# Coloquinte/sleekit

Measured on AMD Instinct MI355X. Metric: Mweights/sec quantized (GPTQ 3-bit, 4096x4096 layer), higher is better.
Workload: dtype f64; 1 GPU; 8 layers 4096x4096, 8-level uniform codebook (GPTQ 3-bit), act_order=diag, damp=0.01, local-search moves=0, layer error included; distinct_inputs=8, allocator_settle_steps=15, gpu_max_hw_queues=4

## Files before the change

include/sleekit_amd.h:

```cpp
#ifndef SLEEKIT_AMD_H
#define SLEEKIT_AMD_H

#include <stddef.h>
#include <stdint.h>

#ifdef __cplusplus
extern "C" {
#endif

#define SLK_OK 0
#define SLK_E_ARG (-1)
#define SLK_E_NOT_PD (-2)
#define SLK_E_HIP (-3)
#define SLK_E_WS (-4)
#define SLK_INFO_HANDOFF_TIMEOUT 0x7fffffff

#define SLK_CB_VALUE 0
#define SLK_CB_INDEX 1
#define SLK_CB_UP 2
#define SLK_CB_DOWN 3
#define SLK_CB_INDEX16 4
#define SLK_CB_INDEX32 5

#define SLK_ORDER_NONE 0
#define SLK_ORDER_DIAG 1
#define SLK_ORDER_ERR 2
#define SLK_ORDER_SQERR 3
#define SLK_ORDER_KEYS 4

typedef void *slk_stream_t;

int slk_abi_version(void);
const char *slk_last_error(void);
int slk_set_option(const char *name, int value);
int slk_get_option(const char *name);
size_t slk_workspace_bytes(int R, int n);

int slk_codebook_apply(const float *x, size_t count, int levels, double lo, double hi, const float *table,
                       int what, void *out, slk_stream_t stream);

size_t slk_codebook_stats_workspace_bytes(void);
int slk_codebook_stats(const float *x, size_t count, int levels, double lo, double hi, const float *table, int by_position,
                       long long *counts, double *sums, double *sqerr, void *workspace, size_t ws_bytes, slk_stream_t stream);
size_t slk_sort_workspace_bytes(size_t count);
int slk_sort_f32(const float *x, size_t count, float *out, void *workspace, size_t ws_bytes, slk_stream_t stream);
int slk_unique_f32(const float *sorted, size_t count, float *out, int *n_out, void *workspace, size_t ws_bytes,
                   slk_stream_t stream);

int slk_rows_divide(const float *x, const float *scale, int R, int n, int invert, float *out,
                    slk_stream_t stream);

int slk_stack_rows(const float *const *src, int batch, int rows, int rows_padded, int cols, float fill, float *dst,
                   slk_stream_t stream);

int slk_hessian_strip_mean(const float *H, const float *mean, int n, float *out,
                           slk_stream_t stream);

int slk_hessian_patch_dead(float *H, float *W, int R, int n, void *workspace, size_t ws_bytes,
                           slk_stream_t stream);

int slk_hessian_accumulate(float *H, float *mean, const float *X, int n, int T,
                           long long count_before, void *workspace, size_t ws_bytes, slk_stream_t stream);

int slk_column_miss(const float *W, int R, int n, int levels, double lo, double hi, const float *table,
                    int squared, float *miss, slk_stream_t stream);

int slk_hessian_prepare(const float *H, int n, float damp, int order_mode, const float *miss,
                        long long *order_out, double *A, void *workspace, size_t ws_bytes,
                        slk_stream_t stream);
int slk_inverse_diag_keys(const double *U, const float *H, int n, float damp, int combined, double *keys,
                          void *workspace, size_t ws_bytes, slk_stream_t stream);
int slk_pivot_keys(const float *H, int n, float damp, double *keys, void *workspace, size_t ws_bytes,
                   slk_stream_t stream);
int slk_factor_ld(int n);
int slk_factor_load(const double *M, int n, double *A, slk_stream_t stream);

int slk_chol_inverse_upper(double *A, int n, double *U, int *info, void *workspace,
                           size_t ws_bytes, slk_stream_t stream);
int slk_chol_inverse_upper_lookahead(double *A, int n, double *U, int *info, void *workspace,
                                     size_t ws_bytes, slk_stream_t stream);
int slk_release_helpers(void);

int slk_hessian_prepare_batch(const float *const *H, int batch, int n, float damp, int order_mode,
                              long long *order_out, double *A, void *workspace, size_t ws_bytes, slk_stream_t stream);
int slk_chol_inverse_upper_batch(double *A, int batch, int n, double *U, int *info, void *workspace,
                                 size_t ws_bytes, slk_stream_t stream);
size_t slk_factor_workspace_bytes_batch(int batch, int n);

size_t slk_factor_payload_words(int n);
int slk_factor_pack(const double *U, const long long *order, const int *info, int n, void *payload,
                    slk_stream_t stream);
int slk_factor_unpack(const void *payload, int n, double *U, long long *order, int *info,
                      slk_stream_t stream);
int slk_factor_unpack_upper(const void *payload, int n, double *U, long long *order, int *info,
                            slk_stream_t stream);
int slk_factor_unpack_upper_batch(const void *const *payloads, int batch, int n, double *U, long long *order, int *info,
                                  int *verdict, slk_stream_t stream);

#define SLK_LOOP_UNSCALE 1
#define SLK_LOOP_LATENCY 2
int slk_gptq_quantize(const float *W, const float *scale, const long long *order, const double *U,
                      int R, int n, int levels, double lo, double hi, const float *table, int min_block,
                      int num_blocks, int flags, float *Q, uint8_t *idx, float *E_out, void *workspace,
                      size_t ws_bytes, slk_stream_t stream);

int slk_gptq_quantize_batch(const float *W, const float *scale, const long long *order, const double *U,
                            int batch, int rows_per_layer, int n, int levels, double lo, double hi,
                            const float *table, int min_block, int num_blocks, int flags, float *Q,
                            uint8_t *idx, float *E_out, void *workspace, size_t ws_bytes, slk_stream_t stream);
size_t slk_workspace_bytes_batch(int batch, int rows_per_layer, int n);

int slk_gptq_quantize_batch_error(const float *W, const float *scale, const long long *order, const double *U,
                                  const float *const *H, float damp, int batch, int rows_per_layer, int n, int levels,
                                  double lo, double hi, const float *table, int min_block, int num_blocks, int flags,
                                  float *Q, uint8_t *idx, float *E_out, float *row_err, void *workspace, size_t ws_bytes,
                                  slk_stream_t stream);

int slk_gptq_quantize_grouped(const float *W, const float *gscale, int group_size, const long long *order, const double *U,
                              int R, int n, int levels, double lo, double hi, const float *table, int min_block,
                              int num_blocks, int flags, float *Q, uint8_t *idx, float *E_out, void *workspace,
                              size_t ws_bytes, slk_stream_t stream);
int slk_gptq_quantize_grouped_batch(const float *W, const float *gscale, int group_size, const long long *order, const double *U,
                                    int batch, int rows_per_layer, int n, int levels, double lo, double hi, const float *table,
                                    int min_block, int num_blocks, int flags, float *Q, uint8_t *idx, float *E_out,
                                    void *workspace, size_t ws_bytes, slk_stream_t stream);
int slk_column_miss_grouped(const float *W, const float *gscale, int group_size, int R, int n, int levels, double lo,
                            double hi, const float *table, int squared, float *miss, slk_stream_t stream);
int slk_scale_search_grouped(const float *W, const float *base, const float *factors, int n_factors, const float *hdiag,
                             int group_size, int R, int n, int levels, double lo, double hi, const float *table, float *out,
                             slk_stream_t stream);
int slk_dequantize_grouped(const uint8_t *idx, const float *gscale, int group_size, int R, int n, int levels, double lo,
                           double hi, const float *table, float *Q, slk_stream_t stream);

int slk_gptq_quantize_grouped_asym(const float *W, const float *gscale, const float *goffset, int group_size, const long long *order,
                                   const double *U, int R, int n, int levels, double lo, double hi, const float *table,
                                   int min_block, int num_blocks, int flags, float *Q, uint8_t *idx, float *E_out,
                                   void *workspace, size_t ws_bytes, slk_stream_t stream);
int slk_gptq_quantize_grouped_asym_batch(const float *W, const float *gscale, const float *goffset, int group_size,
                                         const long long *order, const double *U, int batch, int rows_per_layer, int n,
                                         int levels, double lo, double hi, const float *table, int min_block, int num_blocks,
                                         int flags, float *Q, uint8_t *idx, float *E_out, void *workspace, size_t ws_bytes,
                                         slk_stream_t stream);
int slk_column_miss_grouped_asym(const float *W, const float *gscale, const float *goffset, int group_size, int R, int n,
                                 int levels, double lo, double hi, const float *table, int squared, float *miss,
                                 slk_stream_t stream);
int slk_dequantize_grouped_asym(const uint8_t *idx, const float *gscale, const float *goffset, int group_size, int R, int n,
                                int levels, double lo, double hi, const float *table, float *Q, slk_stream_t stream);
int slk_group_midpoints(const float *W, int group_size, int R, int n, float *goffset, float *Wc, slk_stream_t stream);
int slk_group_center(const float *W, const float *goffset, int group_size, int R, int n, float *Wc, slk_stream_t stream);

#define SLK_DTYPE_F32 0
#define SLK_DTYPE_BF16 1
#define SLK_DTYPE_F16 2
int slk_pack_indices(const uint8_t *idx, int R, int n, int bits, uint32_t *words, slk_stream_t stream);
int slk_unpack_indices(const uint32_t *words, int R, int n, int bits, uint8_t *idx, slk_stream_t stream);
int slk_dequantize_packed(const uint32_t *words, int R, int n, int bits, int levels, double lo, double hi, const float *table,
                          const float *scale, const float *gscale, const float *goffset, int group_size, int out_dtype, void *out,
                          slk_stream_t stream);

#define SLK_MX_MAX 0
#define SLK_MX_MSE 1
#define SLK_MX_DIAG 2
int slk_mx_scale_search(const float *W, const float *hdiag, int mode, int R, int n, uint8_t *scales, float *S,
                        slk_stream_t stream);
int slk_mx_pack(const uint8_t *idx, const float *S, int R, int n, uint8_t *codes, uint8_t *scales, int *flag,
                slk_stream_t stream);
int slk_mx_unpack(const uint8_t *codes, const uint8_t *scales, int R, int n, uint8_t *idx, float *S, int *flag,
                  slk_stream_t stream);
int slk_mx_dequantize(const uint8_t *codes, const uint8_t *scales, int R, int n, int out_dtype, void *out, int *flag,
                      slk_stream_t stream);

int slk_mx_quantize_act(const void *X, int x_dtype, int M, int K, uint8_t *a_codes, uint8_t *a_scales, int *flag,
                        slk_stream_t stream);
int slk_mx_dequantize_act(const uint8_t *a_codes, const uint8_t *a_scales, int M, int K, int out_dtype, void *out, int *flag,
                          slk_stream_t stream);
int slk_mx_gemm(const uint8_t *a_codes, const uint8_t *a_scales, const uint8_t *w_codes, const uint8_t *w_scales,
                const float *bias, int M, int N, int K, int out_dtype, void *out, slk_stream_t stream);

int slk_row_errors(const float *W, const float *Q, const float *H, int R, int n, float *row_err,
                   float *G, void *workspace, size_t ws_bytes, slk_stream_t stream);
int slk_row_errors_batch(const float *W, const float *Q, const float *const *H, int batch, int rows_per_layer,
                         int n, const int *symmetric, float *row_err, void *workspace, size_t ws_bytes,
                         slk_stream_t stream);
int slk_symmetry_flag(const float *H, int n, int *flag, slk_stream_t stream);

int slk_local_search(const float *W, float *Q, const float *H, int R, int n, int levels, double lo,
                     double hi, const float *table, int moves, uint8_t *idx, int *trace, float *gains,
                     int gains_mode, float *row_err, void *workspace, size_t ws_bytes, slk_stream_t stream);
int slk_local_search_batch(const float *W, float *Q, const float *const *H, int batch, int rows_per_layer, int n,
                           int levels, double lo, double hi, const float *table, int moves, uint8_t *idx,
                           const int *symmetric, float *row_err, void *workspace, size_t ws_bytes, slk_stream_t stream);
int slk_local_search_grouped(const float *W, float *Q, const float *H, const float *gscale, int group_size, int R, int n,
                             int levels, double lo, double hi, const float *table, int moves, uint8_t *idx, int *trace,
                             float *row_err, void *workspace, size_t ws_bytes, slk_stream_t stream);

int slk_scale_minmax(const float *W, int R, int n, double lo_code, double hi_code, float *scale,
                     slk_stream_t stream);
int slk_scale_norm(const float *W, int R, int n, float *scale, slk_stream_t stream);
int slk_scale_search(const float *W, const float *base, const float *factors, int n_factors,
                     const float *hdiag, int R, int n, int levels, double lo, double hi, const float *table,
                     float *out, slk_stream_t stream);
int slk_search_step(const float *err, float factor, int R, float *best_err, float *best_f, int init,
                    slk_stream_t stream);
int slk_scale_times(const float *a, const float *b, float c, int R, float *out, slk_stream_t stream);

int slk_diag_mean(const float *H, int n, float *out, void *workspace, size_t ws_bytes,
                  slk_stream_t stream);
int slk_probe_mfma_f64(double *sink, int blocks, int iters, slk_stream_t stream);
int slk_probe_mfma_f32(float *sink, int blocks, int iters, slk_stream_t stream);
int slk_probe_mfma_f64_acc(double *sink, int blocks, int iters, int nacc, slk_stream_t stream);
int slk_probe_chain(double *out, int iters, int mode, slk_stream_t stream);
int slk_probe_window_cycles(long long *host_out, int reset);
int slk_probe_panel_cycles(long long *host_out, int reset);
int slk_probe_leaf_chain(double *out, int iters, int waves_per_simd, slk_stream_t stream);

int slk_profile_enable(int on);
int slk_profile_reset(void);
int slk_profile_report(char *buf, size_t cap);

#ifdef __cplusplus
}
#endif
#endif
```

sleekit_amd/_lib.py:

```python

import ctypes
import os
from ctypes import c_char_p, c_double, c_float, c_int, c_longlong, c_size_t, c_void_p

_HERE = os.path.dirname(os.path.abspath(__file__))
LIB_PATH = os.environ.get("SLK_LIB_PATH") or os.path.join(_HERE, "libsleekit_amd.so")

if not os.path.exists(LIB_PATH):
    raise ImportError(
        f"{LIB_PATH} is missing: build it with `make -C sleekit_amd/csrc` "
        "(or `python -c 'import __graft_entry__ as g; g.build()'`). sleekit_amd has no CPU fallback."
    )

lib = ctypes.CDLL(LIB_PATH)

OK, E_ARG, E_NOT_PD, E_HIP, E_WS = 0, -1, -2, -3, -4
CB_VALUE, CB_INDEX, CB_UP, CB_DOWN, CB_INDEX16, CB_INDEX32 = 0, 1, 2, 3, 4, 5
DTYPE_F32, DTYPE_BF16, DTYPE_F16 = 0, 1, 2
MX_MAX, MX_MSE, MX_DIAG = 0, 1, 2
ORDER_NONE, ORDER_DIAG, ORDER_ERR, ORDER_SQERR, ORDER_KEYS = 0, 1, 2, 3, 4
ORDER_MODES = {"none": ORDER_NONE, "diag": ORDER_DIAG, "err": ORDER_ERR, "sqerr": ORDER_SQERR}

P = c_void_p

PROTOTYPES = {
    "slk_abi_version": (c_int, []),
    "slk_last_error": (c_char_p, []),
    "slk_set_option": (c_int, [c_char_p, c_int]),
    "slk_get_option": (c_int, [c_char_p]),
    "slk_workspace_bytes": (c_size_t, [c_int, c_int]),
    "slk_codebook_apply": (c_int, [P, c_size_t, c_int, c_double, c_double, P, c_int, P, P]),
    "slk_rows_divide": (c_int, [P, P, c_int, c_int, c_int, P, P]),
    "slk_stack_rows": (c_int, [P, c_int, c_int, c_int, c_int, c_float, P, P]),
    "slk_hessian_strip_mean": (c_int, [P, P, c_int, P, P]),
    "slk_hessian_patch_dead": (c_int, [P, P, c_int, c_int, P, c_size_t, P]),
    "slk_hessian_accumulate": (c_int, [P, P, P, c_int, c_int, c_longlong, P, c_size_t, P]),
    "slk_codebook_stats_workspace_bytes": (c_size_t, []),
    "slk_codebook_stats": (c_int, [P, c_size_t, c_int, c_double, c_double, P, c_int, P, P, P, P, c_size_t, P]),
    "slk_sort_workspace_bytes": (c_size_t, [c_size_t]),
    "slk_sort_f32": (c_int, [P, c_size_t, P, P, c_size_t, P]),
    "slk_unique_f32": (c_int, [P, c_size_t, P, P, P, c_size_t, P]),
    "slk_column_miss": (c_int, [P, c_int, c_int, c_int, c_double, c_double, P, c_int, P, P]),
    "slk_hessian_prepare": (c_int, [P, c_int, c_float, c_int, P, P, P, P, c_size_t, P]),
    "slk_inverse_diag_keys": (c_int, [P, P, c_int, c_float, c_int, P, P, c_size_t, P]),
    "slk_pivot_keys": (c_int, [P, c_int, c_float, P, P, c_size_t, P]),
    "slk_factor_ld": (c_int, [c_int]),
    "slk_factor_load": (c_int, [P, c_int, P, P]),
    "slk_chol_inverse_upper": (c_int, [P, c_int, P, P, P, c_size_t, P]),
    "slk_chol_inverse_upper_lookahead": (c_int, [P, c_int, P, P, P, c_size_t, P]),
    "slk_release_helpers": (c_int, []),
    "slk_hessian_prepare_batch": (c_int, [P, c_int, c_int, c_float, c_int, P, P, P, c_size_t, P]),
    "slk_chol_inverse_upper_batch": (c_int, [P, c_int, c_int, P, P, P, c_size_t, P]),
    "slk_factor_workspace_bytes_batch": (c_size_t, [c_int, c_int]),
    "slk_factor_payload_words": (c_size_t, [c_int]),
    "slk_factor_pack": (c_int, [P, P, P, c_int, P, P]),
    "slk_factor_unpack": (c_int, [P, c_int, P, P, P, P]),
    "slk_factor_unpack_upper": (c_int, [P, c_int, P, P, P, P]),
    "slk_factor_unpack_upper_batch": (c_int, [P, c_int, c_int, P, P, P, P, P]),
    "slk_gptq_quantize": (
        c_int,
        [P, P, P, P, c_int, c_int, c_int, c_double, c_double, P, c_int, c_int, c_int, P, P, P, P, c_size_t, P],
    ),
    "slk_gptq_quantize_batch": (
        c_int,
        [P, P, P, P, c_int, c_int, c_int, c_int, c_double, c_double, P, c_int, c_int, c_int, P, P, P, P, c_size_t, P],
    ),
    "slk_workspace_bytes_batch": (c_size_t, [c_int, c_int, c_int]),
    "slk_gptq_quantize_batch_error": (
        c_int,
        [P, P, P, P, P, c_float, c_int, c_int, c_int, c_int, c_double, c_double, P, c_int, c_int, c_int, P, P, P, P, P, c_size_t, P],
    ),
    "slk_gptq_quantize_grouped": (
        c_int,
        [P, P, c_int, P, P, c_int, c_int, c_int, c_double, c_double, P, c_int, c_int, c_int, P, P, P, P, c_size_t, P],
    ),
    "slk_gptq_quantize_grouped_batch": (
        c_int,
        [P, P, c_int, P, P, c_int, c_int, c_int, c_int, c_double, c_double, P, c_int, c_int, c_int, P, P, P, P, c_size_t, P],
    ),
    "slk_column_miss_grouped": (c_int, [P, P, c_int, c_int, c_int, c_int, c_double, c_double, P, c_int, P, P]),
    "slk_scale_search_grouped": (c_int, [P, P, P, c_int, P, c_int, c_int, c_int, c_int, c_double, c_double, P, P, P]),
    "slk_dequantize_grouped": (c_int, [P, P, c_int, c_int, c_int, c_int, c_double, c_double, P, P, P]),
    "slk_gptq_quantize_grouped_asym": (
        c_int,
        [P, P, P, c_int, P, P, c_int, c_int, c_int, c_double, c_double, P, c_int, c_int, c_int, P, P, P, P, c_size_t, P],
    ),
    "slk_gptq_quantize_grouped_asym_batch": (
        c_int,
        [P, P, P, c_int, P, P, c_int, c_int, c_int, c_int, c_double, c_double, P, c_int, c_int, c_int, P, P, P, P, c_size_t, P],
    ),
    "slk_column_miss_grouped_asym": (c_int, [P, P, P, c_int, c_int, c_int, c_int, c_double, c_double, P, c_int, P, P]),
    "slk_dequantize_grouped_asym": (c_int, [P, P, P, c_int, c_int, c_int, c_int, c_double, c_double, P, P, P]),
    "slk_group_midpoints": (c_int, [P, c_int, c_int, c_int, P, P, P]),
    "slk_group_center": (c_int, [P, P, c_int, c_int, c_int, P, P]),
    "slk_pack_indices": (c_int, [P, c_int, c_int, c_int, P, P]),
    "slk_unpack_indices": (c_int, [P, c_int, c_int, c_int, P, P]),
    "slk_dequantize_packed": (c_int, [P, c_int, c_int, c_int, c_int, c_double, c_double, P, P, P, P, c_int, c_int, P, P]),
    "slk_mx_scale_search": (c_int, [P, P, c_int, c_int, c_int, P, P, P]),
    "slk_mx_pack": (c_int, [P, P, c_int, c_int, P, P, P, P]),
    "slk_mx_unpack": (c_int, [P, P, c_int, c_int, P, P, P, P]),
    "slk_mx_dequantize": (c_int, [P, P, c_int, c_int, c_int, P, P, P]),
    "slk_mx_quantize_act": (c_int, [P, c_int, c_int, c_int, P, P, P, P]),
    "slk_mx_dequantize_act": (c_int, [P, P, c_int, c_int, c_int, P, P, P]),
    "slk_mx_gemm": (c_int, [P, P, P, P, P, c_int, c_int, c_int, c_int, P, P]),
    "slk_row_errors": (c_int, [P, P, P, c_int, c_int, P, P, P, c_size_t, P]),
    "slk_row_errors_batch": (c_int, [P, P, P, c_int, c_int, c_int, P, P, P, c_size_t, P]),
    "slk_symmetry_flag": (c_int, [P, c_int, P, P]),
    "slk_local_search": (c_int, [P, P, P, c_int, c_int, c_int, c_double, c_double, P, c_int, P, P, P, c_int, P, P, c_size_t, P]),
    "slk_local_search_batch": (c_int, [P, P, P, c_int, c_int, c_int, c_int, c_double, c_double, P, c_int, P, P, P, P, c_size_t, P]),
    "slk_local_search_grouped": (
        c_int, [P, P, P, P, c_int, c_int, c_int, c_int, c_double, c_double, P, c_int, P, P, P, P, c_size_t, P],
    ),
    "slk_scale_minmax": (c_int, [P, c_int, c_int, c_double, c_double, P, P]),
    "slk_scale_norm": (c_int, [P, c_int, c_int, P, P]),
    "slk_scale_search": (c_int, [P, P, P, c_int, P, c_int, c_int, c_int, c_double, c_double, P, P, P]),
    "slk_search_step": (c_int, [P, c_float, c_int, P, P, c_int, P]),
    "slk_scale_times": (c_int, [P, P, c_float, c_int, P, P]),
    "slk_diag_mean": (c_int, [P, c_int, P, P, c_size_t, P]),
    "slk_probe_mfma_f64": (c_int, [P, c_int, c_int, P]),
    "slk_probe_mfma_f32": (c_int, [P, c_int, c_int, P]),
    "slk_probe_mfma_f64_acc": (c_int, [P, c_int, c_int, c_int, P]),
    "slk_probe_chain": (c_int, [P, c_int, c_int, P]),
    "slk_probe_window_cycles": (c_int, [P, c_int]),
    "slk_probe_panel_cycles": (c_int, [P, c_int]),
    "slk_probe_leaf_chain": (c_int, [P, c_int, c_int, P]),
    "slk_profile_enable": (c_int, [c_int]),
    "slk_profile_reset": (c_int, []),
    "slk_profile_report": (c_int, [c_char_p, c_size_t]),
}


def profile_report():
    import json

    need = lib.slk_profile_report(None, 0)
    buf = ctypes.create_string_buffer(need + 1)
    lib.slk_profile_report(buf, need + 1)
    return json.loads(buf.value.decode())

for _name, (_res, _args) in PROTOTYPES.items():
    _fn = getattr(lib, _name)
    _fn.restype = _res
    _fn.argtypes = _args


def set_option(name, value):
    check(lib.slk_set_option(name.encode(), int(value)))


class option:

    def __init__(self, name, value):
        self.name, self.value = name, value

    def __enter__(self):
        self.old = lib.slk_get_option(self.name.encode())
        set_option(self.name, self.value)
        return self

    def __exit__(self, *exc):
        set_option(self.name, self.old)
        return False


class SleekitAmdError(RuntimeError):
    pass


def check(rc):
    if rc == OK:
        return
    msg = (lib.slk_last_error() or b"").decode("utf-8", "replace")
    if rc == E_ARG:
        raise RuntimeError(msg or "invalid argument")
    raise SleekitAmdError(f"libsleekit_amd error {rc}: {msg}")
```

sleekit_amd/csrc/common.h:

```cpp
#pragma once

#include <hip/hip_runtime.h>
#include <stddef.h>
#include <stdint.h>
#include <stdio.h>

#include "../../include/sleekit_amd.h"

namespace slk {

void set_error(const char *fmt, ...);

#define SLK_REQUIRE(cond, ...)          \
    do {                                \
        if (!(cond)) {                  \
            slk::set_error(__VA_ARGS__); \
            return SLK_E_ARG;           \
        }                               \
    } while (0)

#define SLK_HIP(call)                                                                  \
    do {                                                                               \
        hipError_t e_ = (call);                                                        \
        if (e_ != hipSuccess) {                                                        \
            slk::set_error("%s failed: %s (%s:%d)", #call, hipGetErrorString(e_), __FILE__, __LINE__); \
            return SLK_E_HIP;                                                          \
        }                                                                              \
    } while (0)

#define SLK_LAUNCH_CHECK() SLK_HIP(hipGetLastError())

struct ProfScope {
    int slot;
    hipStream_t stream;
    ProfScope(const char *name, double flops, double bytes, hipStream_t s);
    ~ProfScope();
};

void prof_next_width(long workgroups);

#define SLK_RUN(name, flops, bytes, stream, ...)                 \
    do {                                                         \
        {                                                        \
            slk::ProfScope prof_scope_(name, flops, bytes, stream); \
            __VA_ARGS__;                                         \
        }                                                        \
        SLK_LAUNCH_CHECK();                                      \
    } while (0)

#define SLK_RUN_W(name, flops, bytes, wgs, stream, ...) \
    do {                                                \
        slk::prof_next_width((long)(wgs));              \
        SLK_RUN(name, flops, bytes, stream, __VA_ARGS__); \
    } while (0)

enum Opt {
    OPT_NO_FAST_LEAF,
    OPT_NO_DEFER,
    OPT_NO_WINDOW2,
    OPT_WIN_DBG,
    OPT_NO_REGULAR_SEARCH,
    OPT_NO_FAST_SEARCH_DIV,
    OPT_NO_ERROR_SPLITK,
    OPT_ERROR_CB,
    OPT_NO_SYM_ERROR,
    OPT_NO_BF16_ERROR,
    OPT_NO_BF16_DMA,
    OPT_NO_BF16_HESSIAN,
    OPT_ERROR_F32_BELOW,
    OPT_NO_BF16_ASYM,
    OPT_NO_SYM_AVERAGE,
    OPT_NO_WAVE_SEARCH,
    OPT_LOOKAHEAD,
    OPT_WINDOW_ROWS,
    OPT_PANEL_SPLIT,
    OPT_ROWS_BELOW_WIDE,
    OPT_NO_LOOP_ERROR,
    OPT_COUNT
};
int opt(Opt o);

struct Helper {
    hipStream_t stream;
    hipStream_t stream2;
    hipEvent_t *events;
};
constexpr int HELPER_EVENTS = 512;
hipError_t helper_for(hipStream_t main, int need, Helper *out);

hipError_t lds_opt_in(const void *kernel, size_t bytes);
#define SLK_LDS_OPT_IN(kernel, bytes) SLK_HIP(slk::lds_opt_in(reinterpret_cast<const void *>(kernel), (bytes)))

struct PtrTable {
    const float *p[64];
};

int row_errors_products(const float *W, const float *Q, const float *const *Hs, int batch, int rpl, int n, const int *sym_known,
                        float *row_err, float *G, void *workspace, size_t ws_bytes, slk_stream_t stream);

int loop_error_means(const float *const *Hs, int batch, int n, float *out, hipStream_t s);

static inline hipStream_t as_stream(slk_stream_t s) { return reinterpret_cast<hipStream_t>(s); }

static inline size_t align_up(size_t x, size_t a) { return (x + a - 1) / a * a; }

struct Arena {
    char *base;
    size_t size, used;
    Arena(void *p, size_t bytes) : base(static_cast<char *>(p)), size(bytes), used(0) {}
    template <class T>
    T *take(size_t count) {
        size_t off = align_up(used, 256);
        size_t end = off + count * sizeof(T);
        if (end > size || base == nullptr) return nullptr;
        used = end;
        return reinterpret_cast<T *>(base + off);
    }
};

struct Grid {
    float zero, step, top;
    const float *table;
    int n;
};

static inline Grid make_grid(int levels, double lo, double hi, const float *table = nullptr) {
    Grid g;
    g.zero = (float)lo;
    g.step = (float)((hi - lo) / (double)(levels - 1));
    g.top = (float)(levels - 1);
    g.table = table;
    g.n = levels;
    return g;
}

__device__ __forceinline__ float grid_pos(float x, const Grid g, float shift, float first, float last) {
    float t = (x - g.zero) / g.step;
    t = t + shift;
    t = rintf(t);
    return fminf(fmaxf(t, first), last);
}
__device__ __forceinline__ float grid_val(float t, const Grid g) { return t * g.step + g.zero; }
__device__ __forceinline__ float grid_value(float x, const Grid g) {
    return grid_val(grid_pos(x, g, 0.0f, 0.0f, g.top), g);
}

__device__ __forceinline__ int table_index(float x, const Grid g) {
    const float *lim = g.table + g.n;
    int lo = 0, hi = g.n - 1;
    while (lo < hi) {
        const int mid = (lo + hi) >> 1;
        if (lim[mid] <= x) lo = mid + 1; else hi = mid;
    }
    return lo;
}
__device__ __forceinline__ float cb_value(float x, const Grid g) { return g.table ? g.table[table_index(x, g)] : grid_value(x, g); }
__device__ __forceinline__ int cb_index(float x, const Grid g) {
    return g.table ? table_index(x, g) : (int)grid_pos(x, g, 0.0f, 0.0f, g.top);
}
__device__ __forceinline__ float cb_up(float x, const Grid g) {
    return g.table ? g.table[min(table_index(x, g) + 1, g.n - 1)] : grid_val(grid_pos(x, g, 1.0f, 1.0f, g.top), g);
}
__device__ __forceinline__ float cb_down(float x, const Grid g) {
    return g.table ? g.table[max(table_index(x, g) - 1, 0)] : grid_val(grid_pos(x, g, -1.0f, 0.0f, g.top - 1.0f), g);
}
__device__ __forceinline__ float cb_entry(int k, const Grid g) { return g.table ? g.table[k] : grid_val((float)k, g); }

template <bool OFFSET>
struct GroupQ {
    float s, rs, o;
    __device__ __forceinline__ static GroupQ of(float s, float o = 0.0f) { return {s, 1.0f / s, o}; }
    __device__ __forceinline__ static GroupQ at(const float *S, const float *O, size_t k) {
        GroupQ e = of(S[k]);
        if constexpr (OFFSET) e.o = O[k];
        return e;
    }
    __device__ __forceinline__ float scaled(float x) const {
        if constexpr (OFFSET) return (x - o) / s;
        else return x / s;
    }
    __device__ __forceinline__ float dequant(float v) const {
        if constexpr (OFFSET) return v / rs + o;
        else return v / rs;
    }
    __device__ __forceinline__ float value(float x, const Grid g) const { return dequant(cb_value(scaled(x), g)); }
    __device__ __forceinline__ int index(float x, const Grid g) const { return cb_index(scaled(x), g); }
    __device__ __forceinline__ float up(float x, const Grid g) const { return dequant(cb_up(scaled(x), g)); }
    __device__ __forceinline__ float down(float x, const Grid g) const { return dequant(cb_down(scaled(x), g)); }
};

template <int CTRL>
__device__ __forceinline__ float dpp_f(float x) {
    return __int_as_float(__builtin_amdgcn_update_dpp(0, __float_as_int(x), CTRL, 0xf, 0xf, true));
}
template <int CTRL>
__device__ __forceinline__ int dpp_i(int x) {
    return __builtin_amdgcn_update_dpp(0, x, CTRL, 0xf, 0xf, true);
}
constexpr int DPP_XOR1 = 0xB1, DPP_XOR2 = 0x4E, DPP_HALF_MIRROR = 0x141, DPP_MIRROR = 0x140;

enum { PK_F32 = 0, PK_BF16 = 1, PK_F16 = 2 };

__device__ __forceinline__ unsigned short pk_bf16(float f) {
    const unsigned u = __float_as_uint(f);
    if ((u & 0x7fffffffu) > 0x7f800000u) return 0x7fc0;
    return (unsigned short)((u + 0x7fffu + ((u >> 16) & 1u)) >> 16);
}

template <int OUT>
struct PkOut;
template <>
struct PkOut<PK_F32> {
    typedef float T;
    typedef float V __attribute__((ext_vector_type(4)));
    static __device__ __forceinline__ float cvt(float v) { return v; }
};
template <>
struct PkOut<PK_BF16> {
    typedef unsigned short T;
    typedef unsigned short V __attribute__((ext_vector_type(4)));
    static __device__ __forceinline__ unsigned short cvt(float v) { return pk_bf16(v); }
};
template <>
struct PkOut<PK_F16> {
    typedef _Float16 T;
    typedef _Float16 V __attribute__((ext_vector_type(4)));
    static __device__ __forceinline__ _Float16 cvt(float v) { return (_Float16)v; }
};

__device__ __forceinline__ double readlane_f64(double v, int src) {
    const long long b = __double_as_longlong(v);
    const unsigned lo = (unsigned)__builtin_amdgcn_readlane((int)(b & 0xffffffffLL), src);
    const unsigned hi = (unsigned)__builtin_amdgcn_readlane((int)(b >> 32), src);
    return __longlong_as_double((long long)(((unsigned long long)hi << 32) | lo));
}

__global__ __launch_bounds__(256) static void k_zero_words(unsigned *__restrict__ p, size_t words) {
    for (size_t i = (size_t)blockIdx.x * blockDim.x + threadIdx.x; i < words; i += (size_t)gridDim.x * blockDim.x) p[i] = 0u;
}
__global__ __launch_bounds__(256) static void k_copy_words(unsigned *__restrict__ dst, const unsigned *__restrict__ src, size_t words) {
    for (size_t i = (size_t)blockIdx.x * blockDim.x + threadIdx.x; i < words; i += (size_t)gridDim.x * blockDim.x) dst[i] = src[i];
}
static inline void zero_async(void *p, size_t bytes, hipStream_t s) {
    const size_t words = bytes / 4;
    const int blocks = (int)((words + 1023) / 1024 < 2048 ? (words + 1023) / 1024 : 2048);
    if (words) k_zero_words<<<blocks ? blocks : 1, 256, 0, s>>>(static_cast<unsigned *>(p), words);
}
static inline void copy_async(void *dst, const void *src, size_t bytes, hipStream_t s) {
    const size_t words = bytes / 4;
    const int blocks = (int)((words + 1023) / 1024 < 2048 ? (words + 1023) / 1024 : 2048);
    if (words) k_copy_words<<<blocks ? blocks : 1, 256, 0, s>>>(static_cast<unsigned *>(dst), static_cast<const unsigned *>(src), words);
}

}
```

sleekit_amd/csrc/gptq.hip:

```cpp
#include <stdlib.h>
#include <string.h>

#include <vector>

#include "window2.h"

namespace slk {

constexpr int OP_LEAF = 0, OP_UPDATE = 1;
constexpr int MAX_OPS = 60;

struct Op {
    int kind, a, b, c;
    int m;
    int nl;
};
struct OpTable {
    int count;
    Op op[MAX_OPS];
};

constexpr int PERM_MAX = 16384;

template <bool LDS>
__device__ __forceinline__ void stage_row(float *rowbuf, const float *src, int n) {
    if constexpr (LDS) {
        __syncthreads();
        for (int c = threadIdx.x; c < (n >> 2); c += 256) reinterpret_cast<float4v_t *>(rowbuf)[c] = reinterpret_cast<const float4v_t *>(src)[c];
        __syncthreads();
    }
}
template <int V>
__device__ __forceinline__ void load_elems(const float *p, float (&v)[V]) {
    if constexpr (V == 4) {
        const float4v_t x = *reinterpret_cast<const float4v_t *>(p);
        v[0] = x[0], v[1] = x[1], v[2] = x[2], v[3] = x[3];
    } else {
        v[0] = *p;
    }
}
template <int V>
__device__ __forceinline__ void store_elems(float *p, const float (&v)[V]) {
    if constexpr (V == 4) *reinterpret_cast<float4v_t *>(p) = (float4v_t){v[0], v[1], v[2], v[3]};
    else *p = v[0];
}

template <bool LDS>
__global__ __launch_bounds__(256) void k_permute_in(const float *__restrict__ W, const float *__restrict__ scale,
                                                    const long long *__restrict__ order, int R, int n,
                                                    float *__restrict__ Qp, int *__restrict__ inv_order, int rpl) {
    extern __shared__ __attribute__((aligned(16))) float rowbuf[];
    constexpr int V = LDS ? 4 : 1;
    const int t = threadIdx.x;
    for (int r = blockIdx.x; r < R; r += gridDim.x) {
        const float *src = W + (size_t)r * n;
        const long long *ord = (LDS || order) ? order + (size_t)(r / rpl) * n : nullptr;
        stage_row<LDS>(rowbuf, src, n);
        const float s = scale ? scale[r] : 1.0f;
        for (int c = V * t; c < n; c += V * 256) {
            long long from[V];
            float v[V];
#pragma unroll
            for (int e = 0; e < V; ++e) from[e] = (LDS || ord) ? ord[c + e] : c + e;
#pragma unroll
            for (int e = 0; e < V; ++e) {
                const float x = LDS ? rowbuf[from[e]] : src[from[e]];
                v[e] = scale ? x / s : x;
            }
            store_elems<V>(Qp + (size_t)r * n + c, v);
        }
    }
    for (int b = blockIdx.x; b < (R + rpl - 1) / rpl; b += gridDim.x)
        for (int c = t; c < n; c += 256) inv_order[(size_t)b * n + (order ? order[(size_t)b * n + c] : c)] = c;
}

struct RowErrArgs {
    const float *W, *E, *scale, *hmean;
    float damp;
    float *row_err;
};
__device__ __forceinline__ double wave_sum_f64(double v) {
#pragma unroll
    for (int off = 32; off > 0; off >>= 1) v += __shfl_down(v, off, 64);
    return v;
}
__device__ __forceinline__ void row_error_store(double se, double sd, double *red, const RowErrArgs &a, int r, int rpl) {
    se = wave_sum_f64(se);
    sd = wave_sum_f64(sd);
    const int t = threadIdx.x;
    if ((t & 63) == 0) {
        red[t >> 6] = se;
        red[4 + (t >> 6)] = sd;
    }
    __syncthreads();
    if (t == 0) {
        const double SE = ((red[0] + red[1]) + red[2]) + red[3], SD = ((red[4] + red[5]) + red[6]) + red[7];
        const double s = a.scale ? (double)a.scale[r] : 1.0;
        const float lambda = a.damp * a.hmean[64 * (r / rpl)];
        a.row_err[r] = (float)((s * s) * SE - (double)lambda * SD);
    }
    __syncthreads();
}

template <bool LDS, bool ERR>
__global__ __launch_bounds__(256) void k_permute_out(const float *__restrict__ Qp, const int *__restrict__ inv_order,
                                                     int R, int n, Grid g, const float *__restrict__ unscale,
                                                     float *__restrict__ Q, uint8_t *__restrict__ idx, int rpl, RowErrArgs ea) {
    extern __shared__ __attribute__((aligned(16))) float rowbuf[];
    __shared__ double red[ERR ? 8 : 1];
    constexpr int V = LDS ? 4 : 1;
    for (int r = blockIdx.x; r < R; r += gridDim.x) {
        const float *src = Qp + (size_t)r * n;
        const int *inv_o = inv_order + (size_t)(r / rpl) * n;
        stage_row<LDS>(rowbuf, src, n);
        const float inv = unscale ? 1.0f / unscale[r] : 1.0f;
        double se = 0.0, sd = 0.0;
        for (int j = V * threadIdx.x; j < n; j += V * 256) {
            float qw[V];
            unsigned packed = 0;
#pragma unroll
            for (int e = 0; e < V; ++e) {
                const float v = LDS ? rowbuf[inv_o[j + e]] : src[inv_o[j + e]];
                if (idx) packed |= (unsigned)(cb_index(v, g) & 255) << (8 * e);
                qw[e] = unscale ? v / inv : v;
            }
            store_elems<V>(Q + (size_t)r * n + j, qw);
            if (idx) {
                if constexpr (LDS) *reinterpret_cast<unsigned *>(idx + (size_t)r * n + j) = packed;
                else idx[(size_t)r * n + j] = (uint8_t)packed;
            }
            if constexpr (ERR) {
                float w[V], ev[V];
                load_elems<V>(ea.W + (size_t)r * n + j, w);
                load_elems<V>(ea.E + (size_t)r * n + j, ev);
#pragma unroll
                for (int e = 0; e < V; ++e) {
                    const float d = w[e] - qw[e];
                    sd += (double)d * (double)d;
                    se += (double)ev[e] * (double)ev[e];
                }
            }
        }
        if constexpr (ERR) row_error_store(se, sd, red, ea, r, rpl);
    }
}
template <class K, class... A>
static int launch_permute(const char *name, double flops, double bytes, K kernel, bool lds, int R, int n, hipStream_t s, A... args) {
    if (lds) SLK_LDS_OPT_IN(kernel, PERM_MAX * 4);
    SLK_RUN(name, flops, bytes, s, kernel<<<R < 2048 ? R : 2048, 256, lds ? (size_t)n * 4 : 0, s>>>(args...));
    return SLK_OK;
}

__global__ __launch_bounds__(256) void k_group_of_column(const long long *__restrict__ order, int batch, int n, int gsize,
                                                         int *__restrict__ pg) {
    const size_t total = (size_t)batch * n;
    for (size_t e = (size_t)blockIdx.x * blockDim.x + threadIdx.x; e < total; e += (size_t)gridDim.x * blockDim.x)
        pg[e] = (int)((order ? order[e] : (long long)e) / gsize);
}

template <bool OFFSET = false>
__global__ __launch_bounds__(256) void k_permute_out_grouped(const float *__restrict__ Qp, const int *__restrict__ inv_order,
                                                             int R, int n, Grid g, const float *__restrict__ S, int gsize,
                                                             float *__restrict__ Q, uint8_t *__restrict__ idx, int rpl,
                                                             const float *__restrict__ O) {
    const int G = n / gsize;
    for (int r = blockIdx.x; r < R; r += gridDim.x) {
        const float *src = Qp + (size_t)r * n;
        const int *inv_o = inv_order + (size_t)(r / rpl) * n;
        for (int j = threadIdx.x; j < n; j += blockDim.x) {
            const float v = src[inv_o[j]];
            Q[(size_t)r * n + j] = v;
            if (idx) {
                const GroupQ<OFFSET> gq = GroupQ<OFFSET>::at(S, O, (size_t)r * G + j / gsize);
                int k = gq.index(v, g);
                if constexpr (OFFSET) {
                    auto back = [&](int t) { return __float_as_uint(gq.dequant(cb_entry(t, g))); };
                    if (back(k) != __float_as_uint(v))
                        for (int t = 0; t < g.n; ++t)
                            if (back(t) == __float_as_uint(v)) {
                                k = t;
                                break;
                            }
                }
                idx[(size_t)r * n + j] = (uint8_t)k;
            }
        }
    }
}

struct WindowSmem {
    LeafTables lt[2];
    int odd[2][4];
    float q[RB][WPITCH];
    float e[RB][WPITCH];
    float cbt[512];
};
struct WindowTile {
    WindowSmem &sm;
    int w0;
    __device__ __forceinline__ float *q(int, int row, int col) const { return &sm.q[row][col - w0]; }
    __device__ __forceinline__ const float *e(int, int row, int k) const { return &sm.e[row][k - w0]; }
    __device__ __forceinline__ static bool straight(int) { return true; }
};

template <bool OFFSET>
__device__ __forceinline__ float leaf_group_q(float x, const GroupQ<OFFSET> e, const Grid g, float inv_step) {
    return e.dequant(grid_value_fast(e.scaled(x), g, inv_step));
}

constexpr int GPITCH = WMAX + 32;
struct GroupTile {
    float s[RB][GPITCH];
    float rs[RB][GPITCH];
};
struct LeafTile {
    const GroupTile &gt;
    typedef GroupQ<false> Step;
    __device__ __forceinline__ Step at(int row, int a, int k) const { return {(&gt.s[row][a])[k], (&gt.rs[row][a])[k]}; }
    template <bool FAST>
    __device__ __forceinline__ static float q(float x, Step e, const Grid g, float inv_step) { return leaf_group_q(x, e, g, inv_step); }
};

constexpr int GSLOTS = 384;
struct GroupSlots {
    float s[RB][GSLOTS + 1];
    float rs[RB][GSLOTS + 1];
    float o[RB][GSLOTS + 1];
    int slot[GPITCH];
};
static_assert(sizeof(WindowSmem) + sizeof(GroupSlots) <= 160 * 1024, "the asymmetric window's LDS exceeds a CU's 160 KiB");
struct LeafSlots {
    const GroupSlots &gs;
    typedef GroupQ<true> Step;
    __device__ __forceinline__ Step at(int row, int a, int k) const {
        const int slot = gs.slot[a + k];
        return {gs.s[row][slot], gs.rs[row][slot], gs.o[row][slot]};
    }
    template <bool FAST>
    __device__ __forceinline__ static float q(float x, Step e, const Grid g, float inv_step) { return leaf_group_q(x, e, g, inv_step); }
};

template <class P>
__device__ __forceinline__ void leaf_tile16(WindowSmem &sm, const P &pol, const LeafTables &lt, int wave, int lane, int a_rel, int w,
                                            const Grid g, float inv_step) {
    const int c16 = lane & 15, row = 4 * wave + (lane >> 4);
    const bool m0 = c16 < w, m1 = c16 + 16 < w;
    const float x0 = m0 ? sm.q[row][a_rel + c16] : 0.0f, x1 = m1 ? sm.q[row][a_rel + 16 + c16] : 0.0f;
    float q0 = 0.0f, q1 = 0.0f, e0 = 0.0f, e1 = 0.0f;
    if (w <= 16) leaf_chain16<16, true>(lt, pol, row, a_rel, c16, x0, x1, q0, q1, e0, e1, g, inv_step);
    else leaf_chain16<32, true>(lt, pol, row, a_rel, c16, x0, x1, q0, q1, e0, e1, g, inv_step);
    if (m0) {
        sm.q[row][a_rel + c16] = q0;
        sm.e[row][a_rel + c16] = e0;
    }
    if (m1) {
        sm.q[row][a_rel + 16 + c16] = q1;
        sm.e[row][a_rel + 16 + c16] = e1;
    }
}

template <bool GROUPED, bool OFFSET>
__device__ __forceinline__ float generic_q(float x, const GroupQ<OFFSET> gq, const Grid g) {
    if constexpr (GROUPED) return gq.value(x, g);
    else return cb_value(x, g);
}

template <bool GROUPED, bool OFFSET = false>
__global__ __launch_bounds__(512) void k_gptq_window(float *__restrict__ Qp, float *__restrict__ Eg,
                                                     const double *__restrict__ U, int R, int n, int w0, int w1,
                                                     Grid g, float inv_step, int fast_ok, int dbg, OpTable tab, int rpl,
                                                     const float *__restrict__ Sg, const int *__restrict__ pg, int G,
                                                     const float *__restrict__ Og) {
    static_assert(GROUPED || !OFFSET, "offsets come with group scales");
    extern __shared__ __attribute__((aligned(16))) char smem_raw[];
    WindowSmem &sm = *reinterpret_cast<WindowSmem *>(smem_raw);
    GroupTile &gt = *reinterpret_cast<GroupTile *>(smem_raw + sizeof(WindowSmem));
    GroupSlots &gs = *reinterpret_cast<GroupSlots *>(smem_raw + sizeof(WindowSmem));
    const bool slots = OFFSET && G <= GSLOTS;
    const int t = threadIdx.x, lane = t & 63, wave = t >> 6;
    const bool helper = wave >= 4;
    const int ht = t - 256;
    const int r0 = blockIdx.x * RB;
    U += (size_t)(r0 / rpl) * n * n;
    if constexpr (GROUPED) pg += (size_t)(r0 / rpl) * n;
    if (g.table) {
        for (int i = t; i < 2 * g.n - 1; i += 512) sm.cbt[i] = g.table[i];
        g.table = sm.cbt;
    }
    const int width = w1 - w0;
    Laps laps(dbg);
    auto lap = [&](int slot, int w) { laps.lap(slot, wave == w); };
    const bool vec4 = tile_vec4(Qp, n, w0);
    auto load_cols = [&](int c_lo, int c_hi, int tid, int nth) { load_tile_cols<RB>(sm.q, Qp, r0, R, n, w0, vec4, c_lo, c_hi, tid, nth); };

    double pu[4] = {0.0, 0.0, 0.0, 0.0};
    int fetch_w = 0;
    int next_fetch = 0;
    auto fetch_block = [&]() {
        fetch_w = 0;
        for (; next_fetch < tab.count; ++next_fetch) {
            const Op nx = tab.op[next_fetch];
            const int w = nx.b - nx.a;
            if (nx.kind != OP_LEAF || w > ULEAF) continue;
            fetch_leaf_block(U, n, nx.a, w, ht, pu);
            fetch_w = w;
            ++next_fetch;
            return;
        }
    };
    auto write_block = [&](int buf) {
        const bool any = write_leaf_tables(sm.lt[buf], pu, fetch_w, ht);
        if (lane == 0) sm.odd[buf][wave - 4] = any ? 1 : 0;
    };

    if constexpr (OFFSET) {
        if (slots) {
            for (int e = t; e < RB * (GSLOTS + 1); e += 512) {
                const int r = e / (GSLOTS + 1), k = e % (GSLOTS + 1);
                const bool in = k < G && r0 + r < R;
                const float sv = in ? Sg[(size_t)(r0 + r) * G + k] : 1.0f;
                gs.s[r][k] = sv;
                gs.rs[r][k] = 1.0f / sv;
                gs.o[r][k] = in ? Og[(size_t)(r0 + r) * G + k] : 0.0f;
            }
            for (int c = t; c < GPITCH; c += 512) gs.slot[c] = c < width ? pg[w0 + c] : GSLOTS;
        }
    }
    if constexpr (GROUPED && !OFFSET) {
        for (int e = t; e < RB * GPITCH; e += 512) {
            const int r = e / GPITCH, c = e % GPITCH;
            const float sv = (c < width && r0 + r < R) ? Sg[(size_t)(r0 + r) * G + pg[w0 + c]] : 1.0f;
            gt.s[r][c] = sv;
            gt.rs[r][c] = 1.0f / sv;
        }
    }

    float warm = 0.0f;
    if (!(dbg & 16)) {
        const int per_xcd = max(1, min(32, (int)gridDim.x >> 3));
        const int slice = (blockIdx.x >> 3) % per_xcd;
        const int lpr = (width + 15) >> 4, total = width * lpr;
        const int per_slice = (total + per_xcd - 1) / per_xcd;
        for (int id = slice * per_slice + t; id < min(total, (slice + 1) * per_slice); id += 512) {
            const int row = id / lpr, c0 = (id % lpr) << 4;
            if (c0 + 15 >= row) warm += reinterpret_cast<const float *>(U + (size_t)(w0 + row) * n + w0 + min(c0, width - 1))[0];
        }
    }

    if (helper) fetch_block();
    const int first_end = (tab.op[0].kind == OP_LEAF && !(dbg & 32)) ? tab.op[0].b : w1;
    load_cols(w0, first_end, t, 512);
    int rest_from = first_end;
    if (helper) {
        if (fetch_w) write_block(0);
        fetch_block();
    }
    __syncthreads();
    lap(7, 0);

    TileUpdate<1, WindowTile, false> upd{{sm, w0}, U, n, n <= 16384, lane & 15, lane >> 4};
    bool primed = false;
    auto generic_leaf = [&](int a, int b, bool staged, int buf) {
        const LeafTables &lt = sm.lt[buf];
        const int myrow = 2 * wave + (lane >> 5), l = lane & 31;
        float *qrow = sm.q[myrow], *erow = sm.e[myrow];
        for (int i = a; i < b; ++i) {
            GroupQ<OFFSET> gq = {1.0f, 1.0f, 0.0f};
            if constexpr (OFFSET) {
                if (slots) {
                    const int k = gs.slot[i - w0];
                    gq = {gs.s[myrow][k], gs.rs[myrow][k], gs.o[myrow][k]};
                } else if (r0 + myrow < R) {
                    gq = GroupQ<true>::at(Sg, Og, (size_t)(r0 + myrow) * G + pg[i]);
                }
            } else if constexpr (GROUPED) {
                gq = {gt.s[myrow][i - w0], gt.rs[myrow][i - w0], 0.0f};
            }
            const float x = qrow[i - w0], q = generic_q<GROUPED>(x, gq, g);
            const double uii = staged ? lt.udr[i - a][0] : U[(size_t)i * n + i];
            const double err = (double)(x - q) / uii;
            __syncthreads();
            for (int j = i + 1 + l; j < b; j += 32) {
                const double uij = staged ? lt.u[i - a][j - a] : U[(size_t)i * n + j];
                const double p = err * uij;
                qrow[j - w0] = (float)((double)qrow[j - w0] - p);
            }
            if (l == 0) {
                erow[i - w0] = (float)err;
                qrow[i - w0] = q;
            }
            __syncthreads();
        }
    };

    int pa = 0, pb = 0, pm = 0, pc = 0, pdone = 0, pleaves = 1;
#ifdef SLK_WINDOW_EXPERIMENTS
    const bool no_updates = dbg & 2, no_leaves = dbg & 1, no_leaf_regs = dbg & 4;
#else
    constexpr bool no_updates = false, no_leaves = false, no_leaf_regs = false;
#endif
    int sbuf = 0;

    for (int oi = 0; oi <= tab.count; ++oi) {
        const bool fin = oi == tab.count;
        const Op op = tab.op[fin ? 0 : oi];
        const bool is_leaf = !fin && op.kind == OP_LEAF;
        if (!fin && (is_leaf ? no_leaves : no_updates)) continue;
        const int prem = (pc - pm + 15) / 16 - pdone;
        const int plo = pm + 16 * pdone;
        int ua = 0, ub = 0, ulo = 0, uhi = 0, uwid = wave, unw = 8;
        bool uready = false, redo = false, use_fast = false, staged = false;
        if (is_leaf) {
            const int w = op.b - op.a;
            staged = w <= ULEAF;
            use_fast = staged && fast_ok;
            if (use_fast) use_fast = (sm.odd[sbuf][0] | sm.odd[sbuf][1] | sm.odd[sbuf][2] | sm.odd[sbuf][3]) == 0;
            if constexpr (OFFSET) use_fast = use_fast && slots;
            lap(1, 0);
        }
        const bool rest = (is_leaf || fin) && rest_from < w1;
        if (rest && (helper || !use_fast)) load_cols(rest_from, w1, use_fast ? ht : t, use_fast ? 256 : 512);
        if (rest) rest_from = w1;
        if (is_leaf) {
            if (use_fast) {
                const int take = prem > 0 ? min(prem, ((prem + pleaves - 1) / pleaves + 3) & ~3) : 0;
                if (helper) {
                    if (fetch_w) write_block(sbuf ^ 1);
                    fetch_block();
                    ua = pa, ub = pb, ulo = plo, uhi = min(pc, plo + 16 * take), uwid = wave - 4, unw = 4;
                } else if (oi + 1 < tab.count && tab.op[oi + 1].kind == OP_UPDATE && !no_updates) {
                    const Op nx = tab.op[oi + 1];
                    upd.load_round(nx.a, nx.b, nx.b, nx.m, wave, 0, upd.cur);
                    primed = true;
                }
                pdone += take;
                pleaves = max(1, pleaves - 1);
            } else {
                if (helper && staged) {
                    if (fetch_w) write_block(sbuf ^ 1);
                    fetch_block();
                }
                ua = pa, ub = pb, ulo = plo, uhi = pc;
                pdone += prem;
            }
        } else if (fin) {
            if (prem <= 0 && !rest) break;
            ua = pa, ub = pb, ulo = plo, uhi = pc;
            pdone += prem;
        } else if (prem > 0 && ((op.c > plo && op.b < pc) || op.m < op.c)) {
            ua = pa, ub = pb, ulo = plo, uhi = pc;
            pdone += prem;
            redo = true;
        } else {
            ua = op.a, ub = op.b, ulo = op.b, uhi = op.m, uready = primed;
            primed = false;
            if (op.m < op.c) pa = op.a, pb = op.b, pm = op.m, pc = op.c, pdone = 0, pleaves = max(1, op.nl);
        }
        if (!is_leaf) lap(10, 0);
        if (ulo < uhi) upd.run(ua, ub, ulo, uhi, uwid, unw, uready);
        if (is_leaf) {
            if (use_fast) {
                if (!helper && !no_leaf_regs) {
                    const int w = op.b - op.a;
                    if constexpr (OFFSET) leaf_tile16(sm, LeafSlots{gs}, sm.lt[sbuf], wave, lane, op.a - w0, w, g, inv_step);
                    else if constexpr (GROUPED) leaf_tile16(sm, LeafTile{gt}, sm.lt[sbuf], wave, lane, op.a - w0, w, g, inv_step);
                    else leaf_tile16(sm, LeafRows{}, sm.lt[sbuf], wave, lane, op.a - w0, w, g, inv_step);
                }
                lap(0, 0);
                lap(5, 4);
            } else {
                __syncthreads();
                generic_leaf(op.a, op.b, staged, sbuf);
            }
            if (staged) sbuf ^= 1;
        } else {
            lap(3, 0);
        }
        __syncthreads();
        if (is_leaf) {
            lap(2, 0);
            lap(6, 4);
        } else {
            lap(4, 0);
        }
        if (redo) --oi;
    }

    store_tile<RB>(sm.q, Qp, r0, R, n, w0, width, vec4, t);
    store_tile<RB>(sm.e, Eg, r0, R, n, w0, width, tile_vec4(Eg, n, w0), t);
    if (warm == 1.2345e-30f) g_win_cycles[15] = 1;
    lap(8, 0);
    laps.flush(lane, wave);
}

template <bool GROUPED, bool OFFSET = false>
__global__ __launch_bounds__(512) void k_gptq_wide_leaf(float *__restrict__ Qp, float *__restrict__ Eg, const double *__restrict__ U,
                                                        int R, int n, int a, int b, Grid g, int rpl, const float *__restrict__ Sg,
                                                        const int *__restrict__ pg, int G, const float *__restrict__ Og) {
    static_assert(GROUPED || !OFFSET, "offsets come with group scales");
    const int lane = threadIdx.x & 63, wave = threadIdx.x >> 6, l = lane & 31;
    const int r0 = blockIdx.x * RB, row = r0 + 2 * wave + (lane >> 5);
    const bool live = row < R;
    U += (size_t)(r0 / rpl) * n * n;
    if constexpr (GROUPED) pg += (size_t)(r0 / rpl) * n;
    float *qrow = Qp + (size_t)min(row, R - 1) * n, *erow = Eg + (size_t)min(row, R - 1) * n;
    for (int i = a; i < b; ++i) {
        float q = 0.0f;
        double err = 0.0;
        if (live) {
            GroupQ<OFFSET> gq = {1.0f, 1.0f, 0.0f};
            if constexpr (GROUPED) gq = GroupQ<OFFSET>::at(Sg, Og, (size_t)row * G + pg[i]);
            const float x = qrow[i];
            q = generic_q<GROUPED>(x, gq, g);
            err = (double)(x - q) / U[(size_t)i * n + i];
        }
        __syncthreads();
        if (live) {
            for (int j = i + 1 + l; j < b; j += 32) {
                const double p = err * U[(size_t)i * n + j];
                qrow[j] = (float)((double)qrow[j] - p);
            }
            if (l == 0) {
                erow[i] = (float)err;
                qrow[i] = q;
            }
        }
        __syncthreads();
    }
}

__global__ __launch_bounds__(256) void k_gptq_trailing(float *__restrict__ Qp, const float *__restrict__ Eg,
                                                       const double *__restrict__ U, int R, int n, int ka, int kb,
                                                       int ja, int jb, int vec_ok, int rpl) {
#ifdef SLK_TRAILING_F64_IMAGE
    __shared__ __attribute__((aligned(16))) Tile64Smem sm;
#else
    __shared__ __attribute__((aligned(16))) Tile64SmemAf sm;
#endif
    const int r0 = blockIdx.y * TILE, j0 = ja + blockIdx.x * TILE;
    U += (size_t)(r0 / rpl) * n * n;
    const int t = threadIdx.x;
    Acc64 acc;
    acc.zero();
    const int kend = ka + (kb - ka + KSTEP - 1) / KSTEP * KSTEP;
    const int a_row = r0 + (t >> 2), a_k = (t & 3) * 8;
    const int b_k = t >> 3, b_c2 = (t & 7) * 2;
    int k_fast = ka;
    if (vec_ok && r0 + TILE <= R && j0 + TILE <= jb) {
        k_fast = ka + (kb - ka) / KSTEP * KSTEP;
        const float *pe = Eg + (size_t)a_row * n + a_k;
        const double *pu = U + (size_t)b_k * n + j0 + b_c2;
        tile64_mac<true, float>(
            acc, sm, ka, k_fast, [&](int k0, float(&v)[8]) { load8f<true>(pe + k0, v); },
            [&](int k0, double(&v)[8]) { load8d_cols(pu + (size_t)k0 * n, v); });
    }
    if (k_fast < kend) {
        const bool row_ok = a_row < R;
        const float *pe = Eg + (size_t)min(a_row, R - 1) * n;
        tile64_mac<true, float>(
            acc, sm, k_fast, kend,
            [&](int k0, float(&v)[8]) {
                const int k = k0 + a_k;
                load8f_guarded(pe + min(k, kb - 1), kb - 1 - k, row_ok, v);
            },
            [&](int k0, double(&v)[8]) {
                const int k = k0 + b_k;
                load8d_cols_guarded(U + (size_t)min(k, kb - 1) * n + j0, b_c2, jb - 1 - j0, k < kb, v);
            });
    }
    if (r0 + TILE <= R && j0 + TILE <= jb) {
        float *q0 = Qp + (size_t)r0 * n + j0;
        float oldq[16];
        int e = 0;
        tile64_foreach(acc, [&](int r, int c, double) { oldq[e++] = q0[(size_t)r * n + c]; });
        e = 0;
        tile64_foreach(acc, [&](int r, int c, double v) { q0[(size_t)r * n + c] = (float)((double)oldq[e++] - v); });
        return;
    }
    tile64_foreach(acc, [&](int r, int c, double v) {
        if (r0 + r < R && j0 + c < jb) {
            float *p = Qp + (size_t)(r0 + r) * n + j0 + c;
            *p = (float)((double)*p - v);
        }
    });
}

static void flatten(int a, int b, int mb, int nb, std::vector<Op> &ops) {
    const int size = b - a;
    if (size <= mb) {
        ops.push_back({OP_LEAF, a, b, 0, 0, 0});
        return;
    }
    int step = (size + nb - 1) / nb;
    if (step < mb) step = mb;
    for (int s = a; s < b; s += step) {
        const int e = s + step < b ? s + step : b;
        flatten(s, e, mb, nb, ops);
        if (e < b) ops.push_back({OP_UPDATE, s, e, b, b, 1});
    }
}

struct Plan {
    struct Step {
        int kind, a, b, c;
        std::vector<Op> ops;
    };
    std::vector<Step> steps;
};

static void plan(int a, int b, int mb, int nb, Plan &p) {
    const int size = b - a;
    std::vector<Op> ops;
    flatten(a, b, mb, nb, ops);
    if (size <= mb || (size <= WMAX && (int)ops.size() <= MAX_OPS)) {
        p.steps.push_back({0, a, b, 0, ops});
        return;
    }
    int step = (size + nb - 1) / nb;
    if (step < mb) step = mb;
    for (int s = a; s < b; s += step) {
        const int e = s + step < b ? s + step : b;
        plan(s, e, mb, nb, p);
        if (e < b) p.steps.push_back({1, s, e, b, {}});
    }
}

static bool as_periods(const std::vector<Op> &ops, int wa, int wb, PeriodTable &pt) {
    pt.count = 0;
    size_t i = 0;
    while (i < ops.size()) {
        if (pt.count == MAXP || ops[i].kind != OP_LEAF) return false;
        Period P = {ops[i].a, ops[i].b - ops[i].a, 0, 0};
        ++i;
        if (i + 1 < ops.size() && ops[i].kind == OP_UPDATE && ops[i].a == P.s && ops[i].b == P.s + P.w1 &&
            ops[i + 1].kind == OP_LEAF && ops[i + 1].a == P.s + P.w1 && ops[i].c == ops[i + 1].b) {
            P.w2 = ops[i + 1].b - ops[i + 1].a;
            i += 2;
        }
        const int K = P.w1 + P.w2;
        if (i < ops.size()) {
            if (ops[i].kind != OP_UPDATE || ops[i].a != P.s || ops[i].b != P.s + K || ops[i].c != wb) return false;
            ++i;
        } else if (P.s + K != wb) {
            return false;
        }
        if (P.w1 > ULEAF || P.w2 > ULEAF || (P.s & 1) || (P.w1 & 1) || (P.w2 & 1) || P.w1 < 2) return false;
        pt.p[pt.count++] = P;
    }
    if (pt.count == 0 || pt.p[0].s != wa) return false;
    for (int k = 0; k + 1 < pt.count; ++k) {
        if (pt.p[k + 1].s != pt.p[k].s + pt.p[k].w1 + pt.p[k].w2) return false;
        pt.p[k].nw = pt.p[k + 1].w1 + pt.p[k + 1].w2;
    }
    return true;
}

}

using namespace slk;

namespace slk {
__global__ void k_probe_leaf(double *out, int iters, int mode, Grid g, float inv_step) {
    extern __shared__ __attribute__((aligned(16))) char smem_raw[];
    WindowSmem &sm = *reinterpret_cast<WindowSmem *>(smem_raw);
    const int t = threadIdx.x, lane = t & 63, wave = t >> 6;
    for (int e = t; e < 32 * 32; e += blockDim.x) {
        const int i = e >> 5, j = e & 31;
        sm.lt[0].u[i][j] = j > i ? 0.01 * ((i * 7 + j * 3) % 11 - 5) : 0.0;
        if (i == j) sm.lt[0].udr[i][0] = 1.0 + 0.01 * i, sm.lt[0].udr[i][1] = 1.0 / (1.0 + 0.01 * i);
    }
    for (int e = t; e < RB * 64; e += blockDim.x) sm.q[e >> 6][e & 63] = 0.37f * ((e * 13) % 17 - 8);
    __syncthreads();
    const long long t0 = (long long)__builtin_readcyclecounter();
    double4_t macc = {0, 0, 0, 0};
    double vacc = 1.0;
    const bool leafer = mode == 4 ? (wave & 2) == 0 : (wave < 4 || mode == 0);
    if (mode == 4) mode = leafer ? 0 : 1;
    if (t == 0) out[2] = (double)__builtin_amdgcn_s_getreg((4 << 11) | (0 << 6) | 4);
    if (leafer || mode == 0) {
        for (int it = 0; it < iters; ++it) leaf_tile16(sm, LeafRows{}, sm.lt[0], ((wave & 1) + ((wave >> 2) << 1)) & 3, lane, (it & 1) * 32, 32, g, inv_step);
    } else if (mode == 5) {
        typedef __bf16 probe_bf16x8_t __attribute__((ext_vector_type(8)));
        typedef float probe_f32x16_t __attribute__((ext_vector_type(16)));
        probe_bf16x8_t av, bv;
        for (int k = 0; k < 8; ++k) av[k] = (__bf16)(1.0f + lane), bv[k] = (__bf16)2.0f;
        probe_f32x16_t c16 = {0, 0, 0, 0, 0, 0, 0, 0, 0, 0, 0, 0, 0, 0, 0, 0};
        for (int it = 0; it < iters * 64; ++it) c16 = __builtin_amdgcn_mfma_f32_32x32x16_bf16(av, bv, c16, 0, 0, 0);
        vacc = c16[0];
    } else if (mode == 1) {
        for (int it = 0; it < iters * 64; ++it) macc = __builtin_amdgcn_mfma_f64_16x16x4f64(1.0 + lane, 2.0, macc, 0, 0, 0);
    } else if (mode == 2) {
        for (int it = 0; it < iters * 400; ++it) vacc = __builtin_fma(vacc, 1.0000001, 1e-9);
    } else {
        for (int it = 0; it < iters * 100; ++it) vacc += sm.lt[1].u[(it + lane) & 31][lane & 31];
    }
    const long long t1 = (long long)__builtin_readcyclecounter();
    __shared__ long long leaf_cycles[16];
    if (lane == 0) leaf_cycles[wave] = leafer || mode == 0 ? t1 - t0 : 0;
    __syncthreads();
    if (t == 0) {
        out[0] = (double)(t1 - t0);
        out[1] = sm.q[3][5] + sm.e[2][7];
        long long slowest = 0;
        for (int w = 0; w < (int)blockDim.x / 64; ++w) slowest = leaf_cycles[w] > slowest ? leaf_cycles[w] : slowest;
        out[3] = (double)slowest;
    }
    if (macc[0] + vacc == 1.2345e-30) out[1] = macc[0];
}
}

extern "C" int slk_probe_leaf_chain(double *out, int iters, int waves_per_simd, slk_stream_t stream) {
    const int mode = waves_per_simd / 10;
    waves_per_simd %= 10;
    SLK_REQUIRE(out && iters > 0 && waves_per_simd >= 1 && waves_per_simd <= 4 && mode >= 0 && mode <= 5, "bad arguments");
    hipStream_t s = as_stream(stream);
    const Grid g = make_grid(8, -1.0, 1.0);
    SLK_HIP(hipFuncSetAttribute(reinterpret_cast<const void *>(k_probe_leaf), hipFuncAttributeMaxDynamicSharedMemorySize,
                                (int)sizeof(WindowSmem)));
    SLK_RUN("probe_leaf", 0, 0, s, k_probe_leaf<<<1, 256 * waves_per_simd, sizeof(WindowSmem), s>>>(out, iters, mode, g, 1.0f / g.step));
    return SLK_OK;
}

extern "C" int slk_probe_window_cycles(long long *host_out, int reset) {
    SLK_REQUIRE(host_out, "null pointer");
    SLK_HIP(hipDeviceSynchronize());
    SLK_HIP(hipMemcpyFromSymbol(host_out, HIP_SYMBOL(g_win_cycles), sizeof(long long) * 16));
    SLK_HIP(hipMemcpyFromSymbol(host_out + 16, HIP_SYMBOL(g_win_trace), sizeof(long long) * 64));
    if (reset) {
        long long zero[64] = {0};
        SLK_HIP(hipMemcpyToSymbol(HIP_SYMBOL(g_win_cycles), zero, sizeof(long long) * 16));
        SLK_HIP(hipMemcpyToSymbol(HIP_SYMBOL(g_win_trace), zero, sizeof(zero)));
    }
    return SLK_OK;
}

extern "C" int slk_gptq_quantize(const float *W, const float *scale, const long long *order, const double *U,
                                 int R, int n, int levels, double lo, double hi, const float *table, int min_block, int num_blocks,
                                 int flags, float *Q, uint8_t *idx, float *E_out, void *workspace, size_t ws_bytes,
                                 slk_stream_t stream) {
    return slk_gptq_quantize_batch(W, scale, order, U, 1, R, n, levels, lo, hi, table, min_block, num_blocks, flags, Q, idx,
                                   E_out, workspace, ws_bytes, stream);
}

template <bool GROUPED, bool OFFSET>
constexpr size_t window_lds() {
    return sizeof(WindowSmem) + (OFFSET ? sizeof(GroupSlots) : GROUPED ? sizeof(GroupTile) : 0);
}
template <bool GROUPED, bool OFFSET>
static int launch_window(double flops, double bytes, int row_tiles, hipStream_t s, float *Qp, float *Eg, const double *U, int R, int n,
                         int w0, int w1, Grid g, float inv_step, int fast_ok, int dbg, const OpTable &tab, int rpl, const float *Sg,
                         const int *pg, int G, const float *Og) {
    if (w1 - w0 > WMAX) {
        SLK_REQUIRE(tab.count == 1 && tab.op[0].kind == OP_LEAF, "a window of %d columns that is not one leaf", w1 - w0);
        SLK_RUN(OFFSET ? "gptq_window_wide_grouped_asym" : GROUPED ? "gptq_window_wide_grouped" : "gptq_window_wide", flops, bytes, s,
                k_gptq_wide_leaf<GROUPED, OFFSET><<<row_tiles, 512, 0, s>>>(Qp, Eg, U, R, n, w0, w1, g, rpl, Sg, pg, G, Og));
        return SLK_OK;
    }
    SLK_RUN(OFFSET ? "gptq_window_grouped_asym" : GROUPED ? "gptq_window_grouped" : "gptq_window", flops, bytes, s,
            k_gptq_window<GROUPED, OFFSET><<<row_tiles, 512, window_lds<GROUPED, OFFSET>(), s>>>(Qp, Eg, U, R, n, w0, w1, g, inv_step, fast_ok, dbg,
                                                                                               tab, rpl, Sg, pg, G, Og));
    return SLK_OK;
}

static int gptq_loop(const float *W, const float *scale, const long long *order, const double *U, int batch, int rows_per_layer,
                     int n, int levels, double lo, double hi, const float *table, int min_block, int num_blocks, int flags,
                     float *Q, uint8_t *idx, float *E_out, void *workspace, size_t ws_bytes, slk_stream_t stream,
                     const float *gscale, int group_size, const float *goffset, const float *const *Hs = nullptr, float damp = 0.0f,
                     float *row_err = nullptr) {
    const bool grouped = gscale != nullptr, asym = goffset != nullptr;
    const int unscale = flags & SLK_LOOP_UNSCALE;
    SLK_REQUIRE(!unscale || scale, "unscale needs the row scales");
    SLK_REQUIRE(rows_per_layer > 0 && n > 0, "empty layer");
    SLK_REQUIRE(batch >= 1 && batch <= 64, "batch must be 1..64");
    SLK_REQUIRE(batch == 1 || rows_per_layer % TILE == 0, "a batch needs rows_per_layer to be a multiple of 64");
    SLK_REQUIRE(batch == 1 || order, "a batch needs the column orders");
    SLK_REQUIRE((long long)batch * rows_per_layer <= 0x7fffffffLL, "too many rows");
    const int R = batch * rows_per_layer, rpl = rows_per_layer;
    SLK_REQUIRE(levels >= 2 && (table || lo < hi), "codebook needs levels >= 2 and lo < hi");
    SLK_REQUIRE(table == nullptr || levels <= 256, "general codebooks hold at most 256 entries");
    SLK_REQUIRE(idx == nullptr || levels <= 256, "uint8 indices need levels <= 256");
    SLK_REQUIRE(min_block >= 1 && num_blocks >= 1, "min_block_size and num_blocks must be >= 1");
    Arena ws(workspace, ws_bytes);
    float *Qp = ws.take<float>((size_t)R * n);
    float *Eg = ws.take<float>((size_t)R * n);
    int *inv_order = ws.take<int>((size_t)batch * n);
    int *pg = grouped ? ws.take<int>((size_t)batch * n) : nullptr;
    float *hmean = row_err ? ws.take<float>(64 * (size_t)batch) : nullptr;
    if (!Qp || !Eg || !inv_order || (grouped && !pg) || (row_err && !hmean)) {
        set_error("workspace too small for a %d x %d layer", R, n);
        return SLK_E_WS;
    }
    hipStream_t s = as_stream(stream);
    const Grid g = make_grid(levels, lo, hi, table);
    const float inv_step = 1.0f / g.step;
    unsigned step_bits;
    memcpy(&step_bits, &g.step, 4);
    const int fast_ok = table == nullptr && (step_bits & 0x7FFFFFu) != 0x7FFFFFu && g.step > 9.0e-13f && g.step < 1.0e12f &&
                        !opt(OPT_NO_FAST_LEAF);
#ifdef SLK_WINDOW_EXPERIMENTS
    const int dbg = opt(OPT_WIN_DBG);
#else
    const int dbg = opt(OPT_WIN_DBG) & (8 | 16 | 32 | 64 | 128);
#endif
    const bool no_defer = opt(OPT_NO_DEFER) != 0;
    if (asym) SLK_LDS_OPT_IN((k_gptq_window<true, true>), (window_lds<true, true>()));
    else if (grouped) SLK_LDS_OPT_IN((k_gptq_window<true, false>), (window_lds<true, false>()));
    else SLK_LDS_OPT_IN((k_gptq_window<false, false>), (window_lds<false, false>()));
    SLK_LDS_OPT_IN(k_gptq_window2<1>, sizeof(Window2SmemT<1>));
    SLK_LDS_OPT_IN(k_gptq_window2<2>, sizeof(Window2SmemT<2>));
    const int window_rows = opt(OPT_WINDOW_ROWS) == 16 || opt(OPT_WINDOW_ROWS) == 32 ? opt(OPT_WINDOW_ROWS)
                                                                                     : (((flags & SLK_LOOP_LATENCY) || R < 2048) ? 16 : 32);
    const bool periods_ok = !grouped && n % 2 == 0 && n <= 16384 && (uintptr_t)U % 16 == 0 && !opt(OPT_NO_WINDOW2) && (dbg & ~(24 | 64 | 128)) == 0;

    const bool perm_lds = order && n % 4 == 0 && n <= PERM_MAX && ((uintptr_t)W | (uintptr_t)Q | (uintptr_t)workspace) % 16 == 0 &&
                          (idx == nullptr || (uintptr_t)idx % 4 == 0);
    {
        const int rc = launch_permute("permute_in", 0, 8.0 * R * n, perm_lds ? k_permute_in<true> : k_permute_in<false>, perm_lds, R, n, s, W, scale,
                                      order, R, n, Qp, inv_order, rpl);
        if (rc != SLK_OK) return rc;
    }

    const int G = grouped ? n / group_size : 0;
    if (grouped)
        SLK_RUN("group_of_column", 0, 12.0 * batch * n, s,
                k_group_of_column<<<(batch * n + 255) / 256, 256, 0, s>>>(order, batch, n, group_size, pg));

    Plan p;
    plan(0, n, min_block, num_blocks, p);
    const int row_tiles = (R + RB - 1) / RB;
    for (const Plan::Step &st : p.steps) {
        if (st.kind == 0) {
            SLK_REQUIRE(st.ops.size() <= (size_t)MAX_OPS, "a window of %d ops (the table holds %d)", (int)st.ops.size(), MAX_OPS);
            OpTable tab;
            tab.count = (int)st.ops.size();
            double fl = 0, ub = 0;
            for (int i = 0; i < tab.count; ++i) {
                const Op &q = tab.op[i] = st.ops[i];
                if (q.kind == OP_LEAF) {
                    const double w = q.b - q.a;
                    fl += w * (w - 1);
                    ub += 4.0 * w * (w + 1);
                } else {
                    fl += 2.0 * (q.b - q.a) * (q.c - q.b);
                    ub += 8.0 * (q.b - q.a) * (q.c - q.b);
                }
            }
            for (int i = 0; i < tab.count; ++i) {
                Op &q = tab.op[i];
                if (q.kind != OP_UPDATE) continue;
                q.m = q.c;
                q.nl = 1;
                if (no_defer) continue;
                int leaves = 0;
                for (int j = i + 1; j < tab.count; ++j) {
                    const Op &x = tab.op[j];
                    if (x.kind == OP_LEAF) ++leaves;
                    if (x.kind == OP_UPDATE && x.c == q.c && x.a == q.b) {
                        q.m = x.b;
                        q.nl = leaves > 0 ? leaves : 1;
                        break;
                    }
                }
            }
            const double wbytes = 12.0 * R * (st.b - st.a) + ub;
            PeriodTable pt;
            if (st.b - st.a <= WMAX && periods_ok && as_periods(st.ops, st.a, st.b, pt)) {
                if (window_rows == 32)
                    SLK_RUN_W("gptq_window", fl * R, wbytes, (R + 2 * RB - 1) / (2 * RB), s,
                              k_gptq_window2<2><<<(R + 2 * RB - 1) / (2 * RB), 512, sizeof(Window2SmemT<2>), s>>>(
                                  Qp, Eg, U, R, n, st.a, st.b, g, inv_step, fast_ok, dbg & (24 | 64 | 128), pt, rpl));
                else
                    SLK_RUN_W("gptq_window", fl * R, wbytes, row_tiles, s,
                              k_gptq_window2<1><<<row_tiles, 512, sizeof(Window2SmemT<1>), s>>>(Qp, Eg, U, R, n, st.a, st.b, g, inv_step,
                                                                                             fast_ok, dbg & 24, pt, rpl));
            }
            else {
                const auto launch = asym ? launch_window<true, true> : grouped ? launch_window<true, false> : launch_window<false, false>;
                const int rc = launch(fl * R, wbytes, row_tiles, s, Qp, Eg, U, R, n, st.a, st.b, g, inv_step, fast_ok, dbg, tab, rpl, gscale, pg, G,
                                      goffset);
                if (rc != SLK_OK) return rc;
            }
        } else {
            const double K = st.b - st.a, N = st.c - st.b;
            const int vec_ok = n % 4 == 0 && st.a % 4 == 0 && st.b % 2 == 0 && (uintptr_t)U % 16 == 0;
            {
                dim3 grid((st.c - st.b + TILE - 1) / TILE, (R + TILE - 1) / TILE);
                SLK_RUN("gptq_trailing", 2.0 * R * K * N, 4.0 * R * K + 8.0 * K * N + 8.0 * R * N, s,
                        k_gptq_trailing<<<grid, 256, 0, s>>>(Qp, Eg, U, R, n, st.a, st.b, st.b, st.c, vec_ok, rpl));
            }
        }
    }
    if (asym)
        SLK_RUN("permute_out_grouped_asym", 0, (idx ? 17.0 : 8.0) * R * n, s,
                k_permute_out_grouped<true><<<R < 2048 ? R : 2048, 256, 0, s>>>(Qp, inv_order, R, n, g, gscale, group_size, Q, idx, rpl,
                                                                               goffset));
    else if (grouped)
        SLK_RUN("permute_out_grouped", 0, (idx ? 13.0 : 8.0) * R * n, s,
                k_permute_out_grouped<<<R < 2048 ? R : 2048, 256, 0, s>>>(Qp, inv_order, R, n, g, gscale, group_size, Q, idx, rpl,
                                                                         nullptr));
    else {
        RowErrArgs ea{};
        if (row_err) {
            const int rc = loop_error_means(Hs, batch, n, hmean, s);
            if (rc != SLK_OK) return rc;
            ea = RowErrArgs{W, Eg, unscale ? scale : nullptr, hmean, damp, row_err};
        }
        const auto kernel = row_err ? (perm_lds ? k_permute_out<true, true> : k_permute_out<false, true>)
                                    : (perm_lds ? k_permute_out<true, false> : k_permute_out<false, false>);
        const int rc = launch_permute(row_err ? "permute_out_error" : "permute_out", row_err ? 4.0 * R * n : 0,
                                      (row_err ? (idx ? 17.0 : 16.0) : (idx ? 9.0 : 8.0)) * R * n, kernel, perm_lds, R, n, s, Qp, inv_order, R, n, g,
                                      unscale ? scale : nullptr, Q, idx, rpl, ea);
        if (rc != SLK_OK) return rc;
    }
    if (E_out) copy_async(E_out, Eg, sizeof(float) * (size_t)R * n, s);
    return SLK_OK;
}

extern "C" int slk_gptq_quantize_batch(const float *W, const float *scale, const long long *order, const double *U,
                                       int batch, int rows_per_layer, int n, int levels, double lo, double hi,
                                       const float *table, int min_block, int num_blocks, int flags, float *Q, uint8_t *idx,
                                       float *E_out, void *workspace, size_t ws_bytes, slk_stream_t stream) {
    SLK_REQUIRE(W && U && Q, "null pointer");
    SLK_REQUIRE((flags & ~(SLK_LOOP_UNSCALE | SLK_LOOP_LATENCY)) == 0, "unknown flags");
    return gptq_loop(W, scale, order, U, batch, rows_per_layer, n, levels, lo, hi, table, min_block, num_blocks, flags, Q, idx, E_out,
                     workspace, ws_bytes, stream, nullptr, 0, nullptr);
}

extern "C" int slk_gptq_quantize_batch_error(const float *W, const float *scale, const long long *order, const double *U,
                                             const float *const *H, float damp, int batch, int rows_per_layer, int n, int levels,
                                             double lo, double hi, const float *table, int min_block, int num_blocks, int flags,
                                             float *Q, uint8_t *idx, float *E_out, float *row_err, void *workspace, size_t ws_bytes,
                                             slk_stream_t stream) {
    SLK_REQUIRE(W && U && Q && H && row_err, "null pointer");
    SLK_REQUIRE((flags & ~(SLK_LOOP_UNSCALE | SLK_LOOP_LATENCY)) == 0, "unknown flags");
    SLK_REQUIRE(batch >= 1 && batch <= 64, "batch must be 1..64");
    for (int b = 0; b < batch; ++b) SLK_REQUIRE(H[b] != nullptr, "null Hessian (layer %d)", b);
    SLK_REQUIRE(scale == nullptr || (flags & SLK_LOOP_UNSCALE),
                "the carried error is that of the de-scaled Q: row scales need SLK_LOOP_UNSCALE");
    return gptq_loop(W, scale, order, U, batch, rows_per_layer, n, levels, lo, hi, table, min_block, num_blocks, flags, Q, idx, E_out,
                     workspace, ws_bytes, stream, nullptr, 0, nullptr, H, damp, row_err);
}

static int check_grouped(bool tables, const float *W, const double *U, const float *Q, int flags, int rows_per_layer, int n, int group_size) {
    SLK_REQUIRE(W && tables && U && Q, "null pointer");
    SLK_REQUIRE((flags & ~SLK_LOOP_LATENCY) == 0, "the grouped loop takes SLK_LOOP_LATENCY only");
    SLK_REQUIRE(rows_per_layer > 0 && n > 0, "empty layer");
    SLK_REQUIRE(group_size >= 1 && n % group_size == 0, "group_size must be >= 1 and divide n (%d columns, group_size %d)", n,
                group_size);
    return SLK_OK;
}

extern "C" int slk_gptq_quantize_grouped_batch(const float *W, const float *gscale, int group_size, const long long *order,
                                               const double *U, int batch, int rows_per_layer, int n, int levels, double lo,
                                               double hi, const float *table, int min_block, int num_blocks, int flags, float *Q,
                                               uint8_t *idx, float *E_out, void *workspace, size_t ws_bytes, slk_stream_t stream) {
    if (const int rc = check_grouped(gscale != nullptr, W, U, Q, flags, rows_per_layer, n, group_size)) return rc;
    return gptq_loop(W, nullptr, order, U, batch, rows_per_layer, n, levels, lo, hi, table, min_block, num_blocks, flags, Q, idx, E_out,
                     workspace, ws_bytes, stream, gscale, group_size, nullptr);
}

extern "C" int slk_gptq_quantize_grouped(const float *W, const float *gscale, int group_size, const long long *order, const double *U,
                                         int R, int n, int levels, double lo, double hi, const float *table, int min_block,
                                         int num_blocks, int flags, float *Q, uint8_t *idx, float *E_out, void *workspace,
                                         size_t ws_bytes, slk_stream_t stream) {
    return slk_gptq_quantize_grouped_batch(W, gscale, group_size, order, U, 1, R, n, levels, lo, hi, table, min_block, num_blocks,
                                           flags, Q, idx, E_out, workspace, ws_bytes, stream);
}

extern "C" int slk_gptq_quantize_grouped_asym_batch(const float *W, const float *gscale, const float *goffset, int group_size,
                                                    const long long *order, const double *U, int batch, int rows_per_layer, int n,
                                                    int levels, double lo, double hi, const float *table, int min_block,
                                                    int num_blocks, int flags, float *Q, uint8_t *idx, float *E_out, void *workspace,
                                                    size_t ws_bytes, slk_stream_t stream) {
    if (const int rc = check_grouped(gscale && goffset, W, U, Q, flags, rows_per_layer, n, group_size)) return rc;
    return gptq_loop(W, nullptr, order, U, batch, rows_per_layer, n, levels, lo, hi, table, min_block, num_blocks, flags, Q, idx, E_out,
                     workspace, ws_bytes, stream, gscale, group_size, goffset);
}

extern "C" int slk_gptq_quantize_grouped_asym(const float *W, const float *gscale, const float *goffset, int group_size,
                                              const long long *order, const double *U, int R, int n, int levels, double lo, double hi,
                                              const float *table, int min_block, int num_blocks, int flags, float *Q, uint8_t *idx,
                                              float *E_out, void *workspace, size_t ws_bytes, slk_stream_t stream) {
    return slk_gptq_quantize_grouped_asym_batch(W, gscale, goffset, group_size, order, U, 1, R, n, levels, lo, hi, table, min_block,
                                                num_blocks, flags, Q, idx, E_out, workspace, ws_bytes, stream);
}
```

sleekit_amd/csrc/window2.h:

```cpp
#pragma once

#include "window_tile.h"

namespace slk {

constexpr int ERING = 128;
constexpr int MAXP = 32;

struct Period {
    int s, w1, w2, nw;
};
struct PeriodTable {
    int count;
    Period p[MAXP];
};

struct LeafTables8 {
    double u[ULEAF][ULEAF];
    double udr[ULEAF][2];
    __device__ __forceinline__ static int col(int j) { return (j & 7) * 4 + (j >> 3); }
};

template <int SETS>
struct Window2SmemT {
    typename std::conditional<SETS == 1, LeafTables, LeafTables8>::type lt[2][2];
    double sblk[SETS == 1 ? 2 : 1][16 * 64];
    double nblk[SETS == 1 ? 2 : 1][64 * 64];
    float q[RB * SETS][WPITCH];
    float e[RB * SETS][ERING + 4];
    int odd[2][2][4];
    int n_done;
    int s_count;
    float cbt[512];
};
using Window2Smem = Window2SmemT<1>;
template <int SETS>
struct Window2Tile {
    Window2SmemT<SETS> &sm;
    int w0;
    __device__ __forceinline__ float *q(int st, int row, int col) const { return &sm.q[RB * st + row][col - w0]; }
    __device__ __forceinline__ const float *e(int st, int row, int k) const { return &sm.e[RB * st + row][(k - w0) & (ERING - 1)]; }
    __device__ __forceinline__ bool straight(int k) const { return ((k - w0) & 31) == 0; }
};

__device__ __forceinline__ void lds_wait_ge(int *counter, int target) {
    while (__hip_atomic_load(counter, __ATOMIC_ACQUIRE, __HIP_MEMORY_SCOPE_WORKGROUP) < target) __builtin_amdgcn_s_sleep(1);
}
__device__ __forceinline__ void lds_signal(int *counter, int lane) {
    __builtin_amdgcn_fence(__ATOMIC_RELEASE, "workgroup");
    if (lane == 0) __hip_atomic_fetch_add(counter, 1, __ATOMIC_RELEASE, __HIP_MEMORY_SCOPE_WORKGROUP);
}

template <int S>
__device__ __forceinline__ float bcast8(float x) {
    int t = __builtin_amdgcn_update_dpp(0, __float_as_int(x), 0x150 + S, 0xf, 0xf, true);
    t = __builtin_amdgcn_update_dpp(t, __float_as_int(x), 0x150 + 8 + S, 0xf, 0xc, false);
    return __int_as_float(t);
}

template <int NSTEP, bool FAST>
__device__ __forceinline__ void leaf_chain8(const LeafTables8 &lt, int sub, float (&x)[4], float (&q)[4], float (&e)[4], const Grid g,
                                            float inv_step) {
    constexpr int NK = NSTEP / 8;
    const double2_t *urow = reinterpret_cast<const double2_t *>(&lt.u[0][4 * sub]);
    double2_t ulo = urow[0], uhi = NK > 2 ? urow[1] : (double2_t){0.0, 0.0};
    double2_t dr = *reinterpret_cast<const double2_t *>(&lt.udr[0][0]);
    static_for<0, NSTEP>([&](auto ic) {
        constexpr int i = decltype(ic)::value;
        constexpr int kk = i >> 3, s = i & 7;
        const double u[4] = {ulo[0], ulo[1], uhi[0], uhi[1]};
        const double uii = dr[0], rii = dr[1];
        if constexpr (i + 1 < NSTEP) {
            constexpr int first = ((i + 1) >> 3) + (((i + 1) & 7) == 7 ? 1 : 0);
            if constexpr (first < 2) ulo = urow[16 * (i + 1)];
            if constexpr (first < NK && NK > 2) uhi = urow[16 * (i + 1) + 1];
            dr = *reinterpret_cast<const double2_t *>(&lt.udr[i + 1][0]);
        }
        if constexpr (NK == 4) asm volatile("" : "+v"(x[0]), "+v"(x[1]), "+v"(x[2]), "+v"(x[3])::"memory");
        else asm volatile("" : "+v"(x[0]), "+v"(x[1])::"memory");
        const float xi = bcast8<s>(x[kk]);
        const double err = chain_err<FAST>(xi, LeafRows::q<FAST>(xi, {}, g, inv_step), uii, rii);
#pragma unroll
        for (int k = kk; k < NK; ++k) {
            if (k == kk && s == 7) continue;
            x[k] = (float)((double)x[k] - err * u[k]);
        }
    });
#pragma unroll
    for (int k = 0; k < NK; ++k) {
        const double2_t d = *reinterpret_cast<const double2_t *>(&lt.udr[sub + 8 * k][0]);
        q[k] = LeafRows::q<FAST>(x[k], {}, g, inv_step);
        e[k] = (float)chain_err<FAST>(x[k], q[k], d[0], d[1]);
    }
}

template <int SETS>
__global__ __launch_bounds__(512) void k_gptq_window2(float *__restrict__ Qp, float *__restrict__ Eg,
                                                      const double *__restrict__ U, int R, int n, int w0, int w1,
                                                      Grid g, float inv_step, int fast_ok, int prof, PeriodTable tab, int rpl) {
    extern __shared__ __attribute__((aligned(16))) char smem_raw[];
    Window2SmemT<SETS> &sm = *reinterpret_cast<Window2SmemT<SETS> *>(smem_raw);
    constexpr int RBX = RB * SETS;
    const int t = threadIdx.x, lane = t & 63, wave = __builtin_amdgcn_readfirstlane(t >> 6);
    Laps laps(prof);
    const bool timing = laps.on;
    long long tper = laps.mark;
    auto lap = [&](int slot) { laps.lap(slot); };
    const bool helper = wave >= 4;
    const int role_wave = wave & 3;
    constexpr int first_helper = 4;
    if (helper && !(prof & (64 | 128))) __builtin_amdgcn_s_setprio(3);
    if (!helper && (prof & 128)) __builtin_amdgcn_s_setprio(3);
    const int ht = role_wave * 64 + lane;
    const int r0 = blockIdx.x * RBX;
    U += (size_t)(r0 / rpl) * n * n;
    const int np = tab.count;
    const int width = w1 - w0;
    if (g.table) {
        for (int i = t; i < 2 * g.n - 1; i += 512) sm.cbt[i] = g.table[i];
        g.table = sm.cbt;
    }
    auto ring = [&](int c) { return (c - w0) & (ERING - 1); };

    const bool vec4 = tile_vec4(Qp, n, w0);
    auto load_cols = [&](int c_lo, int c_hi, int tid, int nth) { load_tile_cols<RBX>(sm.q, Qp, r0, R, n, w0, vec4, c_lo, c_hi, tid, nth); };
    const Period P0 = tab.p[0];
    const int end0 = P0.s + P0.w1 + P0.w2;
    if (SETS == 2 && t == 0) sm.n_done = 0, sm.s_count = 0;

    if (!helper) {
        const int c16 = lane & 15, rg = lane >> 4;
        int row[SETS];
        bool row_live[SETS];
#pragma unroll
        for (int st = 0; st < SETS; ++st) row[st] = RB * st + 4 * role_wave + rg, row_live[st] = r0 + row[st] < R;
        auto local_update = [&](const double *chunks, int src0, int K, int dst0, int N) {
            const int ncg = (N + 15) >> 4, nks = (K + 3) >> 2;
            const int ai = lane & 3, ak = lane >> 4;
            const float *erow[SETS];
            double acc[SETS][4];
#pragma unroll
            for (int st = 0; st < SETS; ++st) {
                erow[st] = &sm.e[RB * st + 4 * role_wave + ai][0];
#pragma unroll
                for (int cg = 0; cg < 4; ++cg) acc[st][cg] = 0.0;
            }
            auto body = [&](auto nks_c, auto ncg_c) {
                constexpr int NKS = decltype(nks_c)::value, NCG = decltype(ncg_c)::value;
#pragma unroll
                for (int ks = 0; ks < NKS; ++ks) {
                    double a[SETS];
#pragma unroll
                    for (int st = 0; st < SETS; ++st) a[st] = (double)erow[st][ring(src0 + 4 * ks + ak)];
#pragma unroll
                    for (int cg = 0; cg < NCG; ++cg) {
                        const double bchunk = chunks[(size_t)(cg * NKS + ks) * 64 + lane];
#pragma unroll
                        for (int st = 0; st < SETS; ++st) acc[st][cg] = __builtin_amdgcn_mfma_f64_4x4x4f64(a[st], bchunk, acc[st][cg], 0, 0, 0);
                    }
                }
            };
            using std::integral_constant;
            if (K == 64 && ncg == 4) body(integral_constant<int, 16>{}, integral_constant<int, 4>{});
            else if (K == 32 && ncg == 2) body(integral_constant<int, 8>{}, integral_constant<int, 2>{});
            else {
                for (int ks = 0; ks < nks; ++ks) {
                    const int kk = src0 + 4 * ks + ak;
                    double a[SETS];
#pragma unroll
                    for (int st = 0; st < SETS; ++st) {
                        const float ev = erow[st][ring(min(kk, src0 + K - 1))];
                        a[st] = kk < src0 + K ? (double)ev : 0.0;
                    }
#pragma unroll
                    for (int cg = 0; cg < 4; ++cg)
                        if (cg < ncg) {
                            const double bchunk = chunks[(size_t)(cg * nks + ks) * 64 + lane];
#pragma unroll
                            for (int st = 0; st < SETS; ++st) acc[st][cg] = __builtin_amdgcn_mfma_f64_4x4x4f64(a[st], bchunk, acc[st][cg], 0, 0, 0);
                        }
                }
            }
#pragma unroll
            for (int st = 0; st < SETS; ++st)
#pragma unroll
                for (int cg = 0; cg < 4; ++cg) {
                    const int col = dst0 + 16 * cg + c16;
                    if (cg < ncg && col < dst0 + N) sm.q[row[st]][col - w0] = (float)((double)sm.q[row[st]][col - w0] - acc[st][cg]);
                }
        };

        load_cols(w0, end0, t, 512);
        __syncthreads();
        lap(0);
        for (int p = 0; p < np; ++p) {
            const Period P = tab.p[p];
            const int par = p & 1;
#pragma unroll 1
            for (int lf = 0; lf < 2; ++lf) {
                const int w = lf ? P.w2 : P.w1;
                if (w == 0) break;
                const int a = lf ? P.s + P.w1 : P.s;
                if (lf) {
                    if (SETS == 2) lds_wait_ge(&sm.s_count, 4 * p);
                    local_update(sm.sblk[SETS == 1 ? par : 0], P.s, P.w1, a, w);
                }
                lap(2);
                const bool fast = fast_ok && (sm.odd[par][lf][0] | sm.odd[par][lf][1] | sm.odd[par][lf][2] | sm.odd[par][lf][3]) == 0;
                if constexpr (SETS == 2) {
                    const auto &lt = sm.lt[par][lf];
                    const int sub = lane & 7, g8 = lane >> 3;
                    const int lrow = RB * (g8 >> 2) + 4 * role_wave + (g8 & 3);
                    const bool live = r0 + lrow < R;
                    float x[4], qv[4], ev[4];
                    bool m[4];
#pragma unroll
                    for (int k = 0; k < 4; ++k) {
                        m[k] = sub + 8 * k < w;
                        x[k] = m[k] ? sm.q[lrow][a - w0 + sub + 8 * k] : 0.0f;
                        qv[k] = ev[k] = 0.0f;
                    }
                    if (!fast) leaf_chain8<32, false>(lt, sub, x, qv, ev, g, inv_step);
                    else if (w <= 16) leaf_chain8<16, true>(lt, sub, x, qv, ev, g, inv_step);
                    else leaf_chain8<32, true>(lt, sub, x, qv, ev, g, inv_step);
#pragma unroll
                    for (int k = 0; k < 4; ++k) {
                        if (m[k]) {
                            const int col = a + sub + 8 * k;
                            sm.q[lrow][col - w0] = qv[k];
                            sm.e[lrow][ring(col)] = ev[k];
                            if (live) Eg[(size_t)(r0 + lrow) * n + col] = ev[k];
                        }
                    }
                } else {
                    const auto &lt = sm.lt[par][lf];
                    const bool m0 = c16 < w, m1 = c16 + 16 < w;
                    const float x0 = m0 ? sm.q[row[0]][a - w0 + c16] : 0.0f, x1 = m1 ? sm.q[row[0]][a - w0 + 16 + c16] : 0.0f;
                    float q0 = 0.0f, q1 = 0.0f, e0 = 0.0f, e1 = 0.0f;
                    if (!fast) leaf_chain16<32, false>(lt, LeafRows{}, 0, 0, c16, x0, x1, q0, q1, e0, e1, g, inv_step);
                    else if (w <= 16) leaf_chain16<16, true>(lt, LeafRows{}, 0, 0, c16, x0, x1, q0, q1, e0, e1, g, inv_step);
                    else leaf_chain16<32, true>(lt, LeafRows{}, 0, 0, c16, x0, x1, q0, q1, e0, e1, g, inv_step);
                    if (m0) {
                        sm.q[row[0]][a - w0 + c16] = q0;
                        sm.e[row[0]][ring(a + c16)] = e0;
                        if (row_live[0]) Eg[(size_t)(r0 + row[0]) * n + a + c16] = e0;
                    }
                    if (m1) {
                        sm.q[row[0]][a - w0 + 16 + c16] = q1;
                        sm.e[row[0]][ring(a + 16 + c16)] = e1;
                        if (row_live[0]) Eg[(size_t)(r0 + row[0]) * n + a + 16 + c16] = e1;
                    }
                }
                lap(1);
            }
            if (timing && lane == 0 && wave == 0) g_win_trace[p] += (long long)__builtin_readcyclecounter() - tper;
            __syncthreads();
            tper = timing ? (long long)__builtin_readcyclecounter() : 0;
            lap(3);
            if (P.nw) local_update(sm.nblk[SETS == 1 ? par : 0], P.s, P.w1 + P.w2, P.s + P.w1 + P.w2, P.nw);
            if (SETS == 2) lds_signal(&sm.n_done, lane);
            lap(2);
        }
    } else {
        double pu[2][4];
        auto fetch_tables = [&](int p) {
            if (p >= np) return;
            const Period P = tab.p[p];
            fetch_leaf_block(U, n, P.s, P.w1, ht, pu[0]);
            fetch_leaf_block(U, n, P.s + P.w1, max(1, P.w2), ht, pu[1]);
        };
        auto write_tables = [&](int p) {
            if (p >= np) return;
            const Period P = tab.p[p];
#pragma unroll
            for (int lf = 0; lf < 2; ++lf) {
                const bool any = write_leaf_tables(sm.lt[p & 1][lf], pu[lf], lf ? P.w2 : P.w1, ht);
                if (lane == 0) sm.odd[p & 1][lf][role_wave] = any ? 1 : 0;
            }
        };
        typedef double double2_t __attribute__((ext_vector_type(2)));
        auto stage_fetch = [&](auto steps_c, double2_t *regs, int a, int K, int lo, int N) {
            constexpr int STEPS = decltype(steps_c)::value;
            const int ncg = (N + 15) >> 4, nks = (K + 3) >> 2, total = ncg * nks;
            const int half = lane >> 5, k = (lane >> 3) & 3, piece = lane & 7;
            int ch = 2 * role_wave + half;
            int cg = ch / nks, ks = ch - cg * nks;
            const double *colp = U + (size_t)a * n + lo;
#pragma unroll
            for (int it = 0; it < STEPS; ++it) {
                const bool over = ch >= total;
                const int cgc = over ? ncg - 1 : cg, ksc = over ? nks - 1 : ks;
                const int row = min(4 * ksc + k, K - 1);
                const int col = min(16 * cgc + 2 * piece, N - 2);
                regs[it] = *reinterpret_cast<const double2_t *>(colp + (size_t)row * n + col);
                ch += 8;
                ks += 8;
                while (ks >= nks) ks -= nks, ++cg;
            }
        };
        auto stage_store = [&](auto steps_c, const double2_t *regs, double *chunks, int K, int N) {
            constexpr int STEPS = decltype(steps_c)::value;
            const int total = ((N + 15) >> 4) * ((K + 3) >> 2);
#pragma unroll
            for (int it = 0; it < STEPS; ++it) {
                const int pr = role_wave + 4 * it;
                if (2 * pr + (lane >> 5) < total) *reinterpret_cast<double2_t *>(chunks + (size_t)pr * 128 + 2 * lane) = regs[it];
            }
        };
        using std::integral_constant;
        const integral_constant<int, 8> steps_n{};
        const integral_constant<int, 2> steps_s{};
        double2_t nreg[8], sreg[2];

        TileUpdate<SETS, Window2Tile<SETS>, true> upd{{sm, w0}, U, n, true, lane & 15, lane >> 4};

        fetch_tables(0);
        load_cols(w0, end0, t, 512);
        if (P0.w2) {
            stage_fetch(steps_s, sreg, P0.s, P0.w1, P0.s + P0.w1, P0.w2);
            stage_store(steps_s, sreg, sm.sblk[0], P0.w1, P0.w2);
        }
        write_tables(0);
        fetch_tables(1);
        __syncthreads();
        lap(0);
        for (int p = 0; p < np; ++p) {
            const Period P = tab.p[p];
            const int K = P.w1 + P.w2;
            if (SETS == 2 && p >= 1) {
                if (P.w2) stage_store(steps_s, sreg, sm.sblk[0], P.w1, P.w2);
                lds_signal(&sm.s_count, lane);
            }
            write_tables(p + 1);
            lap(6);
            if (P.nw) stage_fetch(steps_n, nreg, P.s, K, P.s + K, P.nw);
            const Period N1 = tab.p[min(p + 1, np - 1)];
            const bool has_s = p + 1 < np && N1.w2;
            if (has_s) stage_fetch(steps_s, sreg, N1.s, N1.w1, N1.s + N1.w1, N1.w2);
            lap(4);
            fetch_tables(p + 2);
            lap(10);
            if (p == 0) load_cols(end0, w1, ht, 256);
            lap(11);
            if (p >= 1) {
                const Period M = tab.p[p - 1];
                const int lo = P.s + K;
                if (lo < w1) upd.run(M.s, M.s + M.w1 + M.w2, lo, w1, role_wave, 4, false);
            }
            lap(5);
            if (SETS == 2) lds_wait_ge(&sm.n_done, 4 * p);
            if (P.nw) stage_store(steps_n, nreg, sm.nblk[SETS == 1 ? (p & 1) : 0], K, P.nw);
            if (SETS == 1 && has_s) stage_store(steps_s, sreg, sm.sblk[(p + 1) & 1], N1.w1, N1.w2);
            if (timing && lane == 0 && wave == first_helper) g_win_trace[32 + p] += (long long)__builtin_readcyclecounter() - tper;
            __syncthreads();
            tper = timing ? (long long)__builtin_readcyclecounter() : 0;
            lap(7);
        }
    }

    store_tile<RBX>(sm.q, Qp, r0, R, n, w0, width, vec4, t);
    laps.flush(lane, wave);
}

}
```

sleekit_amd/dist.py:

```python

import operator
import os

import torch
import torch.distributed as dist


always_exchange = False


rehearse = None
_rehearsal_payloads = {}
_stream_pool = {}


class _Done:

    def __init__(self, event=None):
        self.event = event

    def wait(self):
        if self.event is not None:
            torch.cuda.current_stream().wait_event(self.event)
        return True


def world():
    if rehearse is not None:
        return rehearse
    if dist.is_available() and dist.is_initialized():
        return dist.get_rank(), dist.get_world_size()
    return 0, 1


def row_range(R, rank, size):
    base, extra = divmod(R, size)
    lo = rank * base + min(rank, extra)
    return lo, lo + base + (1 if rank < extra else 0)


def factor_root(position, size):
    return position % size


def _layer_kind(layer):
    if layer.get("gscale") is not None:
        return ("group", int(layer["group_size"]))
    return "row" if layer.get("scale") is not None else "unscaled"


def check_layers(layers, moves=0):
    grouped = False
    for l, lay in enumerate(layers):
        if "goffset" in lay:
            raise NotImplementedError(f"layer {l}: group offsets (`goffset`) are not supported in quantize_stream")
        S, g = lay.get("gscale"), lay.get("group_size")
        if S is None and g is None:
            continue
        R, n = lay["W"].shape
        if S is None or g is None:
            raise ValueError(f"layer {l}: group scales need both `gscale` and `group_size`")
        if lay.get("scale") is not None:
            raise ValueError(f"layer {l}: `gscale` and `scale` are exclusive (one scale per row, or per row and group)")
        try:
            g = operator.index(g) if not isinstance(g, bool) else 0
        except TypeError:
            g = 0
        if g < 1 or n % g != 0:
            raise ValueError(f"layer {l}: group_size must be an int >= 1 that divides the {n} columns (got {lay['group_size']!r})")
        if tuple(S.shape) != (R, n // g) or S.dtype != torch.float32:
            raise ValueError(f"layer {l}: gscale must be float32 ({R}, {n // g}) for a ({R}, {n}) layer with group_size {g}; "
                             f"got {S.dtype} {tuple(S.shape)}")
        grouped = True
    if grouped and moves > 0:
        raise NotImplementedError("quantize_stream: local search (nb_ls_moves > 0) is not available with group scales")


def plan_rounds(layers, size, bucket=True):
    n_layers = len(layers)
    if size <= 1 or not bucket:
        groups = [list(range(n_layers))]
    else:
        by_shape = {}
        for l, lay in enumerate(layers):
            key = (tuple(lay["W"].shape), tuple(lay["H"].shape), _layer_kind(lay))
            by_shape.setdefault(key, []).append(l)
        groups = list(by_shape.values())
    rounds, root, position = [], [None] * n_layers, 0
    for members in groups:
        for i in range(0, len(members), max(size, 1)):
            chunk = members[i:i + max(size, 1)]
            for l in chunk:
                root[l] = factor_root(position, max(size, 1))
                position += 1
            rounds.append(chunk)
    return rounds, root


class HipBackend:

    def __init__(self, quantizer, act_order="diag", damp=0.01, nb_ls_moves=0, with_error=True, overlap=True):
        from . import engine

        self.engine, self.quantizer, self.overlap = engine, quantizer, overlap
        self.act_order, self.damp, self.moves, self.with_error = act_order, damp, nb_ls_moves, with_error
        self.local_batch = int(os.environ.get("SLK_LOCAL_BATCH", self.local_batch))
        self.local_batch_cols = int(os.environ.get("SLK_LOCAL_BATCH_COLS", self.local_batch_cols))
        self.group_rows = int(os.environ.get("SLK_GROUP_ROWS", self.group_rows))
        self.short_factor_batch = int(os.environ.get("SLK_SHORT_FACTOR_BATCH", self.short_factor_batch))
        self.short_rows = int(os.environ.get("SLK_SHORT_ROWS", self.short_rows))
        self.group_wide_rows = int(os.environ.get("SLK_GROUP_WIDE_ROWS", self.group_wide_rows))
        self.group_bytes = int(os.environ.get("SLK_GROUP_BYTES", self.group_bytes))

    def streams(self):
        if not self.overlap:
            return None, None, None
        if not hasattr(self, "_streams"):
            nf, nl = (self.overlap if isinstance(self.overlap, tuple) else (3, 1))
            dev_index = torch.cuda.current_device()
            pool = _stream_pool.setdefault(dev_index, [])
            while len(pool) < nf + nl + 1:
                pool.append(torch.cuda.Stream())
            self._streams = (pool[:nf], pool[nf], pool[nf + 1:nf + 1 + nl])
        return self._streams

    def payload_words(self, n):
        from . import _lib

        return int(_lib.lib.slk_factor_payload_words(n)) + 1

    def alloc_payload(self, words, device):
        return torch.empty(words, dtype=torch.int64, device=device)

    def pack(self, factor, words):
        from . import _device as dev
        from . import _lib

        order, U, info = factor[:3]
        n = U.shape[0]
        payload = self.alloc_payload(words, U.device)
        _lib.check(_lib.lib.slk_factor_pack(dev.ptr(U), dev.ptr(order), dev.ptr(info), n, dev.ptr(payload), dev.stream_handle()))
        mark = self.payload_words(n) - 1
        if len(factor) > 3:
            payload[mark:mark + 1].copy_(factor[3])
        else:
            payload[mark:mark + 1].fill_(-1)
        return payload

    def unpack(self, payload, n):
        from . import _device as dev
        from . import _lib

        order = torch.empty(n, dtype=torch.int64, device=payload.device)
        U = torch.empty((n, n), dtype=torch.float64, device=payload.device)
        info = torch.empty(1, dtype=torch.int32, device=payload.device)
        _lib.check(_lib.lib.slk_factor_unpack(dev.ptr(payload), n, dev.ptr(U), dev.ptr(order), dev.ptr(info), dev.stream_handle()))
        mark = self.payload_words(n) - 1
        return order, U, info, payload[mark:mark + 1].to(torch.int32)

    def factorize(self, layer):
        eng = self.engine
        H, n = layer["H"], layer["H"].shape[0]
        miss = eng.sort_keys(layer["W"], H, eng.require_uniform(self.quantizer), self.act_order, self.damp, scale=layer.get("scale"),
                             gscale=layer.get("gscale"), group_size=layer.get("group_size"))
        factor = eng.factorize(H, n, self.damp, eng.order_mode_code(self.act_order), miss)
        if self.with_error:
            factor = factor + (self._symmetry(layer),)
        return factor

    def _plain_order(self):
        from . import _lib

        return self.engine.order_mode_code(self.act_order) in (_lib.ORDER_NONE, _lib.ORDER_DIAG)

    def _symmetry(self, layer):
        if layer.get("symmetric") is True:
            dev_ = layer["H"].device
            if getattr(self, "_yes", None) is None or self._yes.device != dev_:
                self._yes = torch.ones(1, dtype=torch.int32, device=dev_)
            return self._yes
        return self.engine.symmetry_flag(layer["H"])

    def factorize_many(self, layers):
        eng = self.engine
        n = layers[0]["H"].shape[0]
        mode = eng.order_mode_code(self.act_order)
        if not self._plain_order() or any(lay["H"].shape[0] != n for lay in layers) or len(layers) > 64:
            return [self.factorize(lay) for lay in layers]
        order, U, info = eng.factorize_batch([lay["H"] for lay in layers], n, self.damp, mode)
        out = []
        for b, lay in enumerate(layers):
            fac = (order[b], U[b], info[b:b + 1])
            if self.with_error:
                fac = fac + (self._symmetry(lay),)
            out.append(fac)
        return out

    group_rows = 8192
    group_bytes = 1 << 32
    group_wide_rows = 256
    short_factor_batch = 8
    short_rows = 6144

    def group_limit(self, layer, rows):
        if rows <= 0:
            return 0
        if not self.wants_local_batch(layer):
            if not (self.group_wide_rows and rows <= self.group_wide_rows and self._plain_order()):
                return 0
        n = layer["H"].shape[0]
        padded = (rows + 127) // 128 * 128
        return int(min(64, self.group_rows // padded, self.group_bytes // (8 * n * n)))

    def note_statuses(self, infos, layers, defer=False):
        from . import _device as dev

        def label(l):
            R, n = layers[l]["W"].shape
            return f"quantize_stream: layer {l} ({R} x {n}), compute_hessian_chol"

        have = [l for l, info in enumerate(infos) if info is not None]
        if not have:
            return
        if defer or dev.lazy_errors:
            for l in have:
                dev.note_info(infos[l], label(l), defer=True)
            return
        codes = torch.cat([infos[l].reshape(1) for l in have]).cpu().tolist()
        for l, code in zip(have, codes):
            if code != 0:
                dev.raise_not_pd(code, label(l))

    def run_rows(self, layer, lo, hi, factor):
        eng = self.engine
        if hi <= lo:
            n, device = layer["W"].shape[1], layer["W"].device
            return dict(Q=torch.empty((0, n), dtype=torch.float32, device=device), idx=torch.empty((0, n), dtype=torch.uint8, device=device),
                        row_err=torch.empty(0, dtype=torch.float32, device=device) if self.with_error else None, rows=(lo, hi))

        def shard(key):
            return layer[key][lo:hi].contiguous() if layer.get(key) is not None else None

        W, sc, S = shard("W"), shard("scale"), shard("gscale")
        carried = self._carried_error([layer])
        res = eng.quantize_layer(W, layer["H"], self.quantizer, sc, self.act_order, self.damp, self.moves, *self.blocks,
                                 factor=factor[:3], lookahead=not self.overlap, want_ls_error=carried == "search",
                                 want_loop_error=carried == "loop", gscale=S, group_size=layer.get("group_size"))
        err = None
        if res.ls_error is not None:
            err = res.ls_error if sc is None else (res.ls_error * sc) * sc
        elif res.loop_error is not None:
            err = res.loop_error
        elif self.with_error and len(factor) > 3:
            err = eng.row_errors_batch(W[None], res.Q[None], [layer["H"]], factor[3])[0]
        elif self.with_error:
            err = eng.row_errors(W, res.Q, layer["H"])
        return dict(Q=res.Q, idx=res.idx, row_err=err, rows=(lo, hi))

    blocks = (32, 8)

    def _carried_error(self, layers):
        if not self.with_error or layers[0].get("gscale") is not None or not all(lay.get("symmetric") is True for lay in layers):
            return None
        if self.moves > 0:
            return "search"
        return "loop" if self.engine.loop_error_route() else None

    min_batch = 2

    def can_batch(self, round_layers, lo, hi):
        if len(round_layers) < self.min_batch or len(round_layers) > 64 or hi == lo:
            return False
        first = round_layers[0]
        kind = _layer_kind(first)
        return all(lay["W"].shape == first["W"].shape and lay["H"].shape == first["H"].shape
                   and _layer_kind(lay) == kind for lay in round_layers)

    def run_round(self, round_layers, lo, hi, payloads):
        from . import _device as dev
        from . import _lib

        B, n = len(round_layers), round_layers[0]["H"].shape[0]
        device = round_layers[0]["W"].device
        if not hasattr(self, "_ustacks"):
            self._ustacks = {}
        key = (device.index, dev.stream_handle(), n)
        U = self._ustacks.get(key)
        if U is None or U.shape[0] < B:
            U = self._ustacks[key] = torch.zeros((B, n, n), dtype=torch.float64, device=device)
        U = U[:B]
        import ctypes

        order = torch.empty((B, n), dtype=torch.int64, device=device)
        info = torch.empty(B, dtype=torch.int32, device=device)
        known = torch.empty(B, dtype=torch.int32, device=device) if self.with_error else None
        ptrs = (ctypes.c_void_p * B)(*[dev.ptr(p) for p in payloads])
        _lib.check(_lib.lib.slk_factor_unpack_upper_batch(ptrs, B, n, dev.ptr(U), dev.ptr(order), dev.ptr(info), dev.ptr(known),
                                                          dev.stream_handle()))
        return self._run_stacked(round_layers, lo, hi, order, U, info, known)

    local_batch = 8
    local_batch_cols = 1536

    def wants_local_batch(self, layer):
        R, n = layer["W"].shape
        small = n <= self.local_batch_cols or (n <= 2 * self.local_batch_cols and R <= 1024)
        return self.local_batch > 1 and small and self._plain_order()

    def wants_stacked_loop(self, layer):
        R, n = layer["W"].shape
        return self.local_batch > 1 and not self.wants_local_batch(layer) and R <= 2048 and self._plain_order()

    def run_round_stacked(self, round_layers, factors):
        order = _stack_views([f[0] for f in factors])
        U = _stack_views([f[1] for f in factors])
        info = torch.cat([f[2] for f in factors])
        known = torch.cat([f[3] for f in factors]) if all(len(f) > 3 for f in factors) else None
        return self._run_stacked(round_layers, 0, round_layers[0]["W"].shape[0], order, U, info, known)

    def run_round_local(self, round_layers):
        eng = self.engine
        n = round_layers[0]["H"].shape[0]
        order, U, info = eng.factorize_batch([lay["H"] for lay in round_layers], n, self.damp, eng.order_mode_code(self.act_order))
        return self._run_stacked(round_layers, 0, round_layers[0]["W"].shape[0], order, U, info, None)

    def _run_stacked(self, round_layers, lo, hi, order, U, info, known):
        eng = self.engine
        B, n = len(round_layers), round_layers[0]["H"].shape[0]
        device = round_layers[0]["W"].device
        rows = hi - lo
        Rp = (rows + 127) // 128 * 128
        Hs = [lay["H"] for lay in round_layers]

        def stacked(key, fill):
            if round_layers[0].get(key) is None:
                return None
            return eng.stack_rows([lay[key][lo:hi] for lay in round_layers], Rp, fill)

        W, sc, S = stacked("W", 0.0), stacked("scale", 1.0), stacked("gscale", 1.0)
        cb = eng.require_uniform(self.quantizer)
        want_idx = cb[0] <= 256
        carried = self._carried_error(round_layers)
        if self.moves > 0 and S is None:
            Ws = eng.rows_divide(W.view(B * Rp, n), sc.reshape(-1)).view(B, Rp, n) if sc is not None else W
            Q, idx, _, _ = eng.gptq_loop(Ws, cb, order, U, *self.blocks, want_idx=want_idx)
            err = torch.empty((B, Rp), dtype=torch.float32, device=device) if carried == "search" else None
            eng.local_search_batch(Ws, Q, Hs, cb, self.moves, idx if want_idx else None, known, err)
            if sc is not None:
                Q = eng.rows_divide(Q.view(B * Rp, n), sc.reshape(-1), invert=True).view(B, Rp, n)
                if err is not None:
                    err = (err * sc) * sc
        else:
            Q, idx, _, err = eng.gptq_loop(W, cb, order, U, *self.blocks, scale=sc, gscale=S, group_size=round_layers[0].get("group_size"),
                                           want_idx=want_idx, unscale=sc is not None, Hs=Hs if carried == "loop" else None, damp=self.damp)
        if self.with_error and err is None:
            err = eng.row_errors_batch(W, Q, Hs, known)
        return [dict(Q=Q[b, :rows], idx=idx[b, :rows] if want_idx else None, row_err=None if err is None else err[b, :rows], rows=(lo, hi),
                     info=info[b:b + 1]) for b in range(B)]


def _guard_inputs(layers, stream):
    if stream is None:
        return
    for lay in layers:
        for key in ("W", "H", "scale", "gscale", "mean"):
            t = lay.get(key)
            if isinstance(t, torch.Tensor) and t.is_cuda:
                t.record_stream(stream)


def _stack_views(tensors):
    t0 = tensors[0]
    step = t0.numel()
    base = t0.untyped_storage().data_ptr()
    if t0.is_contiguous() and all(t.is_contiguous() and t.shape == t0.shape and t.dtype == t0.dtype and t.untyped_storage().data_ptr() == base
                                  and t.storage_offset() == t0.storage_offset() + i * step for i, t in enumerate(tensors)):
        return t0.as_strided((len(tensors),) + tuple(t0.shape), (step,) + tuple(t0.stride()))
    return torch.stack(tensors)


class _NullCtx:
    def __enter__(self):
        return self

    def __exit__(self, *a):
        return False


def _all_gather_words(payload, size):
    if rehearse is not None:
        ev = None
        if payload.is_cuda:
            ev = torch.cuda.Event()
            ev.record(torch.cuda.current_stream())
        return [payload] * size, _Done(ev)
    if dist.get_backend() == "nccl":
        out = torch.empty(size * payload.numel(), dtype=payload.dtype, device=payload.device)
        work = dist.all_gather_into_tensor(out, payload, async_op=True)
        return list(out.chunk(size)), work
    outs = [torch.empty_like(payload) for _ in range(size)]
    return outs, dist.all_gather(outs, payload, async_op=True)


def _quantize_stream_local(layers, small, short, backend, join):
    n_layers = len(layers)
    out = [None] * n_layers
    fstreams, _, lstreams = backend.streams()
    side = fstreams is not None
    pool = (fstreams + lstreams) if side else [None]
    here = torch.cuda.current_stream() if side else None

    def on(st):
        return torch.cuda.stream(st) if st is not None else _NullCtx()

    def keep(shards, idxs):
        for l, shard in zip(idxs, shards):
            out[l] = shard
            if here is not None:
                for t in shard.values():
                    if isinstance(t, torch.Tensor):
                        t.record_stream(here)

    for st in pool:
        if st is not None:
            st.wait_stream(here)
    if small:
        rounds, _ = plan_rounds([layers[l] for l in small], backend.local_batch)
        for i, members in enumerate(rounds):
            st = pool[i % len(pool)]
            idxs = [small[m] for m in members]
            if not join:
                _guard_inputs([layers[l] for l in idxs], st)
            with on(st):
                if len(idxs) == 1:
                    lay = layers[idxs[0]]
                    fac = backend.factorize(lay)
                    shards = [dict(backend.run_rows(lay, 0, lay["W"].shape[0], fac), info=fac[2])]
                else:
                    shards = backend.run_round_local([layers[l] for l in idxs])
            keep(shards, idxs)
    if short:
        ls = lstreams[0] if side else None
        rotation = getattr(backend, "_factor_rotation", 0) if side else 0
        for members in _short_rounds(layers, short, backend):
            facs, events = [], []
            n_ = layers[members[0]]["H"].shape[0]
            fb = max(1, min(int(getattr(backend, "short_factor_batch", 1)), int(getattr(backend, "group_bytes", 1 << 32)) // (32 * n_ * n_)))
            for i in range(0, len(members), fb):
                job = members[i:i + fb]
                fs = fstreams[rotation % len(fstreams)] if side else None
                rotation += 1
                if not join:
                    _guard_inputs([layers[l] for l in job], fs)
                with on(fs):
                    if len(job) > 1 and hasattr(backend, "factorize_many"):
                        facs.extend(backend.factorize_many([layers[l] for l in job]))
                    elif len(job) > 1:
                        facs.extend(backend.factorize(layers[l]) for l in job)
                    else:
                        facs.append(backend.factorize(layers[job[0]]))
                    if side:
                        ev = torch.cuda.Event()
                        ev.record(fs)
                        events.append(ev)
            if not join:
                _guard_inputs([layers[l] for l in members], ls)
            with on(ls):
                for ev in events:
                    ls.wait_event(ev)
                if len(members) == 1:
                    lay = layers[members[0]]
                    shards = [dict(backend.run_rows(lay, 0, lay["W"].shape[0], facs[0]), info=facs[0][2])]
                else:
                    shards = backend.run_round_stacked([layers[l] for l in members], facs)
                if side:
                    for f in facs:
                        for t in f:
                            t.record_stream(ls)
            keep(shards, members)
        if side:
            backend._factor_rotation = rotation % len(fstreams)
    taken = set(small) | set(short)
    rest = [l for l in range(n_layers) if l not in taken]
    if rest:
        for l, shard in zip(rest, _quantize_stream([layers[l] for l in rest], backend, join=join, _local=False)):
            out[l] = shard
    if join and here is not None:
        for st in pool:
            here.wait_stream(st)
    return out


def _short_rounds(layers, short, backend):
    by_shape = {}
    for l in short:
        by_shape.setdefault((tuple(layers[l]["W"].shape), _layer_kind(layers[l])), []).append(l)
    rounds = []
    for (shape, _), members in by_shape.items():
        per = max(2, min(backend.local_batch, int(getattr(backend, "short_rows", 4096)) // max(shape[0], 1)))
        rounds.extend(members[i:i + per] for i in range(0, len(members), per))
    return rounds


def quantize_stream(layers, backend, comm_device=None, join=True):
    check_layers(layers, getattr(backend, "moves", 0))
    out = _quantize_stream(layers, backend, comm_device, join, True)
    note = getattr(backend, "note_statuses", None)
    if note is not None:
        note([None if shard is None else shard.get("info") for shard in out], layers, defer=not join)
    return out


def _group_rounds(rounds, layers, backend, rank, size):
    limit_of = getattr(backend, "group_limit", None)
    groups, key_now, count, limit = [], None, 0, 0
    for g, members in enumerate(rounds):
        first = layers[members[0]]
        same = len({(tuple(layers[l]["W"].shape), _layer_kind(layers[l])) for l in members}) == 1
        key = (tuple(first["W"].shape), _layer_kind(first)) if same else None
        if limit_of is not None and key is not None and key == key_now and count + len(members) <= limit:
            groups[-1].append(g)
            count += len(members)
            continue
        groups.append([g])
        key_now, count = key, len(members)
        lo, hi = row_range(first["W"].shape[0], 0, size)
        limit = int(limit_of(first, hi - lo)) if (limit_of is not None and key is not None) else 0
    return groups


def _quantize_stream(layers, backend, comm_device=None, join=True, _local=True):
    rank, size = world()
    n_layers = len(layers)
    if size == 1 and not always_exchange and _local and hasattr(backend, "run_round_local"):
        small = [l for l in range(n_layers) if backend.wants_local_batch(layers[l])]
        short = [l for l in range(n_layers) if backend.wants_stacked_loop(layers[l])]
        small, short = (small if len(small) > 1 else []), (short if len(short) > 1 else [])
        if small or short:
            return _quantize_stream_local(layers, small, short, backend, join)
    fstreams, cstream, lstreams = backend.streams() if hasattr(backend, "streams") else (None, None, None)
    side = fstreams is not None
    here = torch.cuda.current_stream() if side else None
    exchange = size > 1 or always_exchange
    rounds, root = plan_rounds(layers, size, bucket=exchange and getattr(backend, "bucket_by_shape", True))
    n_rounds = len(rounds)
    factors = [None] * n_layers
    ready = [None] * n_layers

    def on(stream):
        return torch.cuda.stream(stream) if stream is not None else _NullCtx()

    groups = _group_rounds(rounds, layers, backend, rank, size) if exchange else [[g] for g in range(n_rounds)]
    slot = {}
    for members_g in groups:
        for j, g in enumerate(members_g):
            for l in rounds[g]:
                slot[l] = j

    jobs = []
    for members_g in groups:
        own = [l for g in members_g for l in rounds[g] if root[l] == rank]
        if len(members_g) > 1 and len(own) > 1 and hasattr(backend, "factorize_many"):
            n_ = layers[own[0]]["H"].shape[0]
            cap = max(1, int(getattr(backend, "group_bytes", 1 << 32)) // (32 * n_ * n_))
            jobs.extend(own[i:i + cap] for i in range(0, len(own), cap))
        else:
            jobs.extend([l] for l in own)
    first = getattr(backend, "_factor_rotation", 0) if side else 0
    if side:
        backend._factor_rotation = (first + len(jobs)) % len(fstreams)
    stream_of = {}
    for k, job in enumerate(jobs):
        fs = fstreams[(first + k) % len(fstreams)] if side else None
        if side and k < len(fstreams):
            fs.wait_stream(here)
        if not join:
            _guard_inputs([layers[l] for l in job], fs)
        with on(fs):
            made = backend.factorize_many([layers[l] for l in job]) if len(job) > 1 else [backend.factorize(layers[job[0]])]
            ev = None
            if side:
                ev = torch.cuda.Event()
                ev.record(fs)
        for l, fac in zip(job, made):
            factors[l], ready[l], stream_of[l] = fac, ev, fs
    gathered = [None] * len(groups)
    keep = []
    if exchange:
        if cstream is not None:
            cstream.wait_stream(here)
        with on(cstream):
            for gi, members_g in enumerate(groups):
                members = [l for g in members_g for l in rounds[g]]
                words = max(backend.payload_words(layers[j]["H"].shape[0]) for j in members)
                stride = (words + 1) // 2 * 2 if len(members_g) > 1 else words
                dev_ = comm_device if comm_device is not None else layers[0]["H"].device
                buffer = None if len(members_g) == 1 else backend.alloc_payload(stride * len(members_g), dev_)
                for j, g in enumerate(members_g):
                    own = [l for l in rounds[g] if root[l] == rank]
                    if own:
                        l = own[0]
                        if ready[l] is not None:
                            cstream.wait_event(ready[l])
                        payload = backend.pack(factors[l], words)
                        if side:
                            for t in factors[l]:
                                t.record_stream(cstream)
                    elif rehearse is not None:
                        n_ = layers[rounds[g][0]]["H"].shape[0]
                        if (n_, words) not in _rehearsal_payloads:
                            _rehearsal_payloads[(n_, words)] = backend.pack(backend.factorize(layers[rounds[g][0]]), words)
                        payload = _rehearsal_payloads[(n_, words)]
                    elif buffer is None:
                        payload = backend.alloc_payload(words, dev_).zero_()
                    else:
                        payload = None
                    if buffer is None:
                        buffer = payload
                    elif payload is not None:
                        buffer[j * stride:j * stride + words].copy_(payload)
                log = getattr(backend, "exchange_log", None)
                if log is not None and buffer.is_cuda:
                    e0, e1 = torch.cuda.Event(enable_timing=True), torch.cuda.Event(enable_timing=True)
                    e0.record(torch.cuda.current_stream())
                    parts, work = _all_gather_words(buffer, size)
                    work.wait()
                    e1.record(torch.cuda.current_stream())
                    log.append((e0, e1, buffer.numel() * buffer.element_size() * (size - 1)))
                else:
                    parts, work = _all_gather_words(buffer, size)
                gathered[gi] = (parts, work, words, stride)
                keep.append(buffer)

    def payload_of(gi, l):
        parts, _, words, stride = gathered[gi]
        return parts[root[l]][slot[l] * stride:slot[l] * stride + words]

    out = [None] * n_layers
    if side:
        for st in lstreams:
            st.wait_stream(here)
    batched_rounds = getattr(backend, "_loop_rotation", 0) if side else 0
    for gi, members_g in enumerate(groups):
        members = [l for g in members_g for l in rounds[g]]
        lo, hi = row_range(layers[members[0]]["W"].shape[0], rank, size)
        if exchange and hasattr(backend, "run_round") and backend.can_batch([layers[l] for l in members], lo, hi):
            ls = lstreams[batched_rounds % len(lstreams)] if side else None
            own = [l for l in members if l in stream_of]
            if side and own and getattr(backend, "rounds_on_factor_streams", True):
                ls = stream_of[own[0]]
            batched_rounds += 1
            if side:
                backend._loop_rotation = batched_rounds % len(lstreams)
            if not join:
                _guard_inputs([layers[l] for l in members], ls)
            with on(ls):
                parts, work = gathered[gi][:2]
                work.wait()
                shards = backend.run_round([layers[l] for l in members], lo, hi, [payload_of(gi, l) for l in members])
                if side:
                    for t in parts:
                        t.record_stream(ls)
            for l, shard in zip(members, shards):
                out[l] = shard
            continue
        for l in members:
            layer = layers[l]
            ls = lstreams[l % len(lstreams)] if side else None
            if not join:
                _guard_inputs([layer], ls)
            with on(ls):
                if exchange:
                    parts, work = gathered[gi][:2]
                    work.wait()
                    if factors[l] is None or always_exchange:
                        factors[l] = backend.unpack(payload_of(gi, l), layer["H"].shape[0])
                elif ready[l] is not None:
                    ls.wait_event(ready[l])
                lo, hi = row_range(layer["W"].shape[0], rank, size)
                shard = backend.run_rows(layer, lo, hi, factors[l])
                if side:
                    for t in factors[l]:
                        t.record_stream(ls)
                    if exchange:
                        for t in gathered[gi][0]:
                            t.record_stream(ls)
            shard["info"] = factors[l][2]
            out[l] = shard
    if side:
        if join:
            for st in lstreams + fstreams:
                here.wait_stream(st)
        extra = [(p,) for p in keep if p is not None] + [tuple(g[0]) for g in gathered if g is not None]
        for f in factors + extra:
            for t in f or ():
                t.record_stream(here)
        for shard in out:
            for t in shard.values():
                if isinstance(t, torch.Tensor):
                    t.record_stream(here)
    return out


def verify_exchange(layers, backend, max_rounds=2):
    rank, size = world()
    out = dict(world_size=size, backend=dist.get_backend() if size > 1 and rehearse is None else "none", rounds_checked=0,
               payload_bytes=0, agree=True)
    if size <= 1 or rehearse is not None:
        return out
    rounds, root = plan_rounds(layers, size)
    for members in rounds[:max_rounds]:
        words = max(backend.payload_words(layers[j]["H"].shape[0]) for j in members)
        own = [l for l in members if root[l] == rank]
        payload = backend.pack(backend.factorize(layers[own[0]]), words) if own else backend.alloc_payload(words, layers[0]["H"].device).zero_()
        parts, work = _all_gather_words(payload, size)
        work.wait()
        weight = torch.arange(1, words + 1, dtype=torch.int64, device=payload.device)

        def sums(t):
            return torch.stack([t.sum(), (t * weight).sum()])

        seen = torch.stack([sums(p) for p in parts])
        views = [torch.empty_like(seen) for _ in range(size)]
        dist.all_gather(views, seen)
        views = torch.stack(views).cpu()
        mine = sums(payload).cpu()
        ok = bool(torch.equal(views[rank][rank], mine))
        for src in range(size):
            ok = ok and all(bool(torch.equal(views[viewer][src], views[src][src])) for viewer in range(size))
        out["agree"] = out["agree"] and ok
        out["rounds_checked"] += 1
        out["payload_bytes"] = int(words * 8)
    return out


def layer_error(shards_row_err, R):
    total = shards_row_err.double().sum()
    rank, size = world()
    if size > 1:
        dist.all_reduce(total)
    return total / R
```

sleekit_amd/engine.py:

```python

import ctypes

import torch

from . import _device as dev
from . import _lib
from .codebook import DeviceCodebook

_INVERSE_ORDERS = {"inv_diag": 0, "combined_diag": 1}
_KEY_ORDERS = ("inv_diag", "combined_diag", "pivot")


def order_mode_code(act_order):
    if act_order in _lib.ORDER_MODES:
        return _lib.ORDER_MODES[act_order]
    if act_order in _KEY_ORDERS:
        return _lib.ORDER_KEYS
    raise RuntimeError(f"Invalid act_order value {act_order}")


def inverse_diag_keys(H, n, damp, combined):
    _, U0, info = factorize(H, n, damp, _lib.ORDER_NONE)
    dev.note_info(info, "compute_hessian_chol")
    ws, ws_bytes = dev.workspace(0, n)
    keys = torch.empty(n, dtype=torch.float64, device=H.device)
    _lib.check(
        _lib.lib.slk_inverse_diag_keys(
            dev.ptr(U0), dev.ptr(H), n, float(damp), int(combined), dev.ptr(keys), dev.ptr(ws), ws_bytes, dev.stream_handle()
        )
    )
    return keys


def pivot_keys(H, n, damp):
    ws, ws_bytes = dev.workspace(0, n)
    keys = torch.empty(n, dtype=torch.float64, device=H.device)
    _lib.check(_lib.lib.slk_pivot_keys(dev.ptr(H), n, float(damp), dev.ptr(keys), dev.ptr(ws), ws_bytes, dev.stream_handle()))
    return keys


def order_keys(H, n, damp, act_order):
    if act_order == "pivot":
        return pivot_keys(H, n, damp)
    return inverse_diag_keys(H, n, damp, _INVERSE_ORDERS[act_order])


def require_uniform(quantizer):
    if not isinstance(quantizer, DeviceCodebook):
        raise NotImplementedError(
            "sleekit_amd runs UniformCodebook / Codebook quantizers on the GPU and has no CPU fallback for arbitrary "
            f"callables (got {type(quantizer).__name__})"
        )
    abi = quantizer._abi()
    if len(quantizer) > 256 and abi[3] is not None:
        raise NotImplementedError("general (table) codebooks on the device hold at most 256 entries")
    return abi


class LayerResult:

    __slots__ = ("Q", "idx", "order", "U", "info", "E", "ls_trace", "ls_error", "loop_error", "S", "O", "codes", "scales")

    def __init__(self):
        self.Q = self.idx = self.order = self.U = self.info = self.E = self.ls_trace = self.ls_error = self.loop_error = None
        self.S = self.O = None
        self.codes = self.scales = None


def factorize(H, n, damp, mode, miss=None, keep=None, lookahead=False):
    ws, ws_bytes = dev.workspace(0, n)
    s = dev.stream_handle()
    ld = _lib.lib.slk_factor_ld(n)
    order = torch.empty(n, dtype=torch.int64, device=H.device)
    A = torch.empty(ld * ld, dtype=torch.float64, device=H.device)
    U = torch.empty((n, n), dtype=torch.float64, device=H.device)
    info = torch.empty(1, dtype=torch.int32, device=H.device)
    _lib.check(
        _lib.lib.slk_hessian_prepare(
            dev.ptr(H), n, float(damp), mode, dev.ptr(miss), dev.ptr(order), dev.ptr(A), dev.ptr(ws), ws_bytes, s
        )
    )
    chol = _lib.lib.slk_chol_inverse_upper_lookahead if lookahead else _lib.lib.slk_chol_inverse_upper
    _lib.check(chol(dev.ptr(A), n, dev.ptr(U), dev.ptr(info), dev.ptr(ws), ws_bytes, s))
    return order, U, info


def factorize_batch(Hs, n, damp, mode):
    B = len(Hs)
    device = Hs[0].device
    assert all(H.shape == (n, n) and H.is_contiguous() and H.dtype == torch.float32 for H in Hs)
    ws, ws_bytes = dev.scratch(_lib.lib.slk_factor_workspace_bytes_batch(B, n), "factor_batch")
    s = dev.stream_handle()
    ld = _lib.lib.slk_factor_ld(n)
    order = torch.empty((B, n), dtype=torch.int64, device=device)
    A = torch.empty(B * ld * ld, dtype=torch.float64, device=device)
    U = torch.empty((B, n, n), dtype=torch.float64, device=device)
    info = torch.empty(B, dtype=torch.int32, device=device)
    ptrs = (ctypes.c_void_p * B)(*[dev.ptr(H) for H in Hs])
    _lib.check(_lib.lib.slk_hessian_prepare_batch(ptrs, B, n, float(damp), mode, dev.ptr(order), dev.ptr(A), dev.ptr(ws), ws_bytes, s))
    _lib.check(_lib.lib.slk_chol_inverse_upper_batch(dev.ptr(A), B, n, dev.ptr(U), dev.ptr(info), dev.ptr(ws), ws_bytes, s))
    return order, U, info


def factorize_order_only(H, n, mode, miss=None):
    ws, ws_bytes = dev.workspace(0, n)
    ld = _lib.lib.slk_factor_ld(n)
    order = torch.empty(n, dtype=torch.int64, device=H.device)
    A = torch.empty(ld * ld, dtype=torch.float64, device=H.device)
    _lib.check(
        _lib.lib.slk_hessian_prepare(
            dev.ptr(H), n, 0.0, mode, dev.ptr(miss), dev.ptr(order), dev.ptr(A), dev.ptr(ws), ws_bytes,
            dev.stream_handle(),
        )
    )
    return order, None, None


def loop_error_route():
    return _lib.lib.slk_get_option(b"no_loop_error") == 0


def gptq_loop(W, cb_abi, order, U, min_block, num_blocks, scale=None, gscale=None, group_size=None, goffset=None, want_idx=True,
              want_E=False, unscale=False, latency=False, Hs=None, damp=None):
    lead, n = tuple(W.shape[:-1]), W.shape[-1]
    B, R = lead if len(lead) == 2 else (1,) + lead
    assert W.is_contiguous() and U.shape == lead[:-1] + (n, n) and U.is_contiguous()
    assert order is None or (order.shape == lead[:-1] + (n,) and order.is_contiguous())
    assert scale is None or (gscale is None and scale.shape == lead and scale.is_contiguous())
    assert (gscale is None) == (group_size is None) and (goffset is None or gscale is not None)
    g = 0
    if gscale is not None:
        g = int(group_size)
        assert g >= 1 and n % g == 0 and Hs is None
        assert all(t is None or (t.shape == lead + (n // g,) and t.dtype == torch.float32 and t.is_contiguous()) for t in (gscale, goffset))
    if Hs is not None:
        assert len(Hs) == B and damp is not None and (scale is None or unscale)
        assert all(H.shape == (n, n) and H.dtype == torch.float32 and H.is_contiguous() for H in Hs)
    ws, ws_bytes = dev.workspace(R, n, batch=B, grouped=gscale is not None and len(lead) == 2)
    Q = torch.empty_like(W, dtype=torch.float32)
    idx = torch.empty(W.shape, dtype=torch.uint8, device=W.device) if want_idx else None
    E = torch.empty_like(Q) if want_E else None
    row_err = torch.empty(lead, dtype=torch.float32, device=W.device) if Hs is not None else None
    levels, lo, hi, table = cb_abi
    factor = (dev.ptr(order), dev.ptr(U))
    rest = (B, R, n, levels, lo, hi, dev.ptr(table), int(min_block), int(num_blocks), (1 if unscale else 0) | (2 if latency else 0),
            dev.ptr(Q), dev.ptr(idx), dev.ptr(E))
    end = (dev.ptr(ws), ws_bytes, dev.stream_handle())
    if goffset is not None:
        rc = _lib.lib.slk_gptq_quantize_grouped_asym_batch(dev.ptr(W), dev.ptr(gscale), dev.ptr(goffset), g, *factor, *rest, *end)
    elif gscale is not None:
        rc = _lib.lib.slk_gptq_quantize_grouped_batch(dev.ptr(W), dev.ptr(gscale), g, *factor, *rest, *end)
    elif Hs is not None:
        ptrs = (ctypes.c_void_p * B)(*[dev.ptr(H) for H in Hs])
        rc = _lib.lib.slk_gptq_quantize_batch_error(dev.ptr(W), dev.ptr(scale), *factor, ptrs, float(damp), *rest, dev.ptr(row_err), *end)
    else:
        rc = _lib.lib.slk_gptq_quantize_batch(dev.ptr(W), dev.ptr(scale), *factor, *rest, *end)
    _lib.check(rc)
    return Q, idx, E, row_err


def run_loop(W, scale, order, U, cb_abi, min_block, num_blocks, want_idx=True, want_E=False, unscale=False, latency=False,
             H=None, damp=None):
    out = gptq_loop(W, cb_abi, order, U, min_block, num_blocks, scale=scale, want_idx=want_idx, want_E=want_E, unscale=unscale,
                    latency=latency, Hs=None if H is None else [H], damp=damp)
    return out[:3] if H is None else out


def run_loop_batch(W, scale, order, U, cb_abi, min_block, num_blocks, want_idx=True, unscale=False, Hs=None, damp=None):
    Q, idx, _, row_err = gptq_loop(W, cb_abi, order, U, min_block, num_blocks, scale=scale, want_idx=want_idx, unscale=unscale,
                                   Hs=Hs, damp=damp)
    return (Q, idx) if Hs is None else (Q, idx, row_err)


def row_errors_batch(W, Q, Hs, symmetric=None):
    B, R, n = W.shape
    assert len(Hs) == B and W.is_contiguous() and Q.is_contiguous()
    assert symmetric is None or (symmetric.dtype == torch.int32 and symmetric.numel() == B and symmetric.is_contiguous())
    ws, ws_bytes = dev.workspace(R, n, batch=B)
    out = torch.empty((B, R), dtype=torch.float32, device=W.device)
    ptrs = (ctypes.c_void_p * B)(*[dev.ptr(H) for H in Hs])
    _lib.check(
        _lib.lib.slk_row_errors_batch(dev.ptr(W), dev.ptr(Q), ptrs, B, R, n, dev.ptr(symmetric), dev.ptr(out), dev.ptr(ws), ws_bytes,
                                      dev.stream_handle())
    )
    return out


def symmetry_flag(H):
    flag = torch.empty(1, dtype=torch.int32, device=H.device)
    _lib.check(_lib.lib.slk_symmetry_flag(dev.ptr(H), H.shape[0], dev.ptr(flag), dev.stream_handle()))
    return flag


def local_search(W, Q, H, cb_abi, moves, idx=None, want_trace=False, gains=None, gains_mode=0, row_err=None, gscale=None,
                 group_size=None):
    R, n = W.shape
    levels, lo, hi, table = cb_abi
    ws, ws_bytes = dev.workspace(R, n)
    trace = torch.empty((R, int(moves)), dtype=torch.int32, device=W.device) if want_trace else None
    assert gains is None or (gains.shape == (R, 2, n) and gains.dtype == torch.float32 and gains.is_contiguous())
    if gscale is not None:
        assert gains is None and group_size is not None
        _lib.check(
            _lib.lib.slk_local_search_grouped(
                dev.ptr(W), dev.ptr(Q), dev.ptr(H), dev.ptr(gscale), int(group_size), R, n, levels, lo, hi, dev.ptr(table), int(moves),
                dev.ptr(idx), dev.ptr(trace), dev.ptr(row_err), dev.ptr(ws), ws_bytes, dev.stream_handle(),
            )
        )
        return trace
    _lib.check(
        _lib.lib.slk_local_search(
            dev.ptr(W), dev.ptr(Q), dev.ptr(H), R, n, levels, lo, hi, dev.ptr(table), int(moves), dev.ptr(idx), dev.ptr(trace),
            dev.ptr(gains), int(gains_mode), dev.ptr(row_err), dev.ptr(ws), ws_bytes, dev.stream_handle(),
        )
    )
    return trace


def local_search_batch(W, Q, Hs, cb_abi, moves, idx=None, symmetric=None, row_err=None):
    B, R, n = W.shape
    assert len(Hs) == B and W.is_contiguous() and Q.is_contiguous() and (idx is None or idx.is_contiguous())
    levels, lo, hi, table = cb_abi
    ws, ws_bytes = dev.workspace(R, n, batch=B)
    ptrs = (ctypes.c_void_p * B)(*[dev.ptr(H) for H in Hs])
    _lib.check(
        _lib.lib.slk_local_search_batch(dev.ptr(W), dev.ptr(Q), ptrs, B, R, n, levels, lo, hi, dev.ptr(table), int(moves), dev.ptr(idx),
                                        dev.ptr(symmetric), dev.ptr(row_err), dev.ptr(ws), ws_bytes, dev.stream_handle())
    )


def stack_rows(parts, rows_padded, fill=0.0):
    B = len(parts)
    rows = parts[0].shape[0]
    cols = parts[0].shape[1] if parts[0].dim() == 2 else 1
    for t in parts:
        if t.dtype != torch.float32 or not t.is_contiguous() or t.shape != parts[0].shape:
            raise ValueError("stack_rows wants contiguous float32 shards of one shape")
    out = torch.empty((B, rows_padded, cols) if parts[0].dim() == 2 else (B, rows_padded), dtype=torch.float32, device=parts[0].device)
    ptrs = (ctypes.c_void_p * B)(*[dev.ptr(t) for t in parts])
    _lib.check(_lib.lib.slk_stack_rows(ptrs, B, rows, int(rows_padded), cols, float(fill), dev.ptr(out), dev.stream_handle()))
    return out


def rows_divide(x, scale, invert=False):
    R, n = x.shape
    out = torch.empty_like(x)
    _lib.check(
        _lib.lib.slk_rows_divide(dev.ptr(x), dev.ptr(scale), R, n, 1 if invert else 0, dev.ptr(out), dev.stream_handle())
    )
    return out


def column_miss(W, cb_abi, squared, gscale=None, group_size=None, goffset=None):
    R, n = W.shape
    levels, lo, hi, table = cb_abi
    out = torch.empty(n, dtype=torch.float32, device=W.device)
    rest = (R, n, levels, lo, hi, dev.ptr(table), 1 if squared else 0, dev.ptr(out), dev.stream_handle())
    if goffset is not None:
        rc = _lib.lib.slk_column_miss_grouped_asym(dev.ptr(W), dev.ptr(gscale), dev.ptr(goffset), int(group_size), *rest)
    elif gscale is not None:
        rc = _lib.lib.slk_column_miss_grouped(dev.ptr(W), dev.ptr(gscale), int(group_size), *rest)
    else:
        rc = _lib.lib.slk_column_miss(dev.ptr(W), *rest)
    _lib.check(rc)
    return out


def sort_keys(W, H, cb_abi, act_order, damp, scale=None, gscale=None, group_size=None, goffset=None):
    mode = order_mode_code(act_order)
    if mode == _lib.ORDER_KEYS:
        return order_keys(H, H.shape[0], damp, act_order)
    if mode < _lib.ORDER_ERR:
        return None
    if scale is not None:
        W = rows_divide(W, scale)
    return column_miss(W, cb_abi, mode == _lib.ORDER_SQERR, gscale, group_size, goffset)


def row_errors(W, Q, H, want_G=False):
    R, n = W.shape
    ws, ws_bytes = dev.workspace(R, n)
    out = torch.empty(R, dtype=torch.float32, device=W.device)
    G = torch.empty((R, n), dtype=torch.float32, device=W.device) if want_G else None
    _lib.check(
        _lib.lib.slk_row_errors(
            dev.ptr(W), dev.ptr(Q), dev.ptr(H), R, n, dev.ptr(out), dev.ptr(G), dev.ptr(ws), ws_bytes, dev.stream_handle()
        )
    )
    return (out, G) if want_G else out


def quantize_layer(
    W, H, quantizer, scale=None, act_order="diag", damp=0.01, nb_ls_moves=0, min_block_size=32, num_blocks=8,
    factor=None, unscale=True, want_idx=True, want_ls_trace=False, lookahead=True, want_ls_error=False, want_loop_error=False,
    *, gscale=None, group_size=None, goffset=None,
):
    assert W.ndim == 2
    assert H.ndim == 2
    assert H.shape[0] == H.shape[1]
    assert H.shape[0] == W.shape[1]
    assert min_block_size >= 1
    assert scale is None or gscale is None
    if goffset is not None and nb_ls_moves > 0:
        raise NotImplementedError("local search with group offsets is not supported (nb_ls_moves must be 0)")
    cb_abi = require_uniform(quantizer)
    if cb_abi[0] > 256:
        want_idx = False
    mode = order_mode_code(act_order)
    R, n = W.shape
    res = LayerResult()
    group = dict(gscale=gscale, group_size=group_size)

    need_scaled_copy = scale is not None and (mode in (_lib.ORDER_ERR, _lib.ORDER_SQERR) or nb_ls_moves > 0)
    Ws, loop_scale = (rows_divide(W, scale), None) if need_scaled_copy else (W, scale)

    check_factor = factor is None
    if factor is None:
        miss = sort_keys(Ws, H, cb_abi, act_order, damp, goffset=goffset, **group)
        factor = factorize(H, n, damp, mode, miss, lookahead=lookahead)
    res.order, res.U, res.info = factor[:3]

    fused = loop_scale is not None and unscale and nb_ls_moves == 0
    carried = want_loop_error and nb_ls_moves == 0 and gscale is None and (scale is None or fused)
    res.Q, res.idx, _, res.loop_error = gptq_loop(Ws, cb_abi, res.order, res.U, min_block_size, num_blocks, scale=loop_scale,
                                                  goffset=goffset, want_idx=want_idx, unscale=fused, latency=lookahead,
                                                  Hs=[H] if carried else None, damp=damp, **group)
    if nb_ls_moves > 0:
        if want_ls_error or gscale is not None:
            res.ls_error = torch.empty(R, dtype=torch.float32, device=W.device)
        res.ls_trace = local_search(Ws, res.Q, H, cb_abi, nb_ls_moves, res.idx, want_trace=want_ls_trace, row_err=res.ls_error, **group)
    if scale is not None and unscale and not fused:
        res.Q = rows_divide(res.Q, scale, invert=True)
    if check_factor:
        dev.note_info(res.info, "compute_hessian_chol")
    return res
```

Baseline: 5565 Mweights/s.

## Stack independent same-shape layers into one tall GPTQ loop via per-layer pointer tables

Adds a layer-pointer table (up to 16 layers) so the GPTQ kernels can read W, scale, order and U for several separate layers without copying them into one stacked tensor. The scheduler groups consecutive same-shape layers that carry the error inside the loop (up to four at a time) and runs them as one batched loop call. The aim is to replace many small per-layer launches, and the serial latency between them, with fewer and taller launches that fill more of the GPU. In exchange, each kernel does extra pointer indirection per row tile, and the layers in a stack must wait for each other's factors before starting.

```diff
diff --git a/include/sleekit_amd.h b/include/sleekit_amd.h
--- a/include/sleekit_amd.h
+++ b/include/sleekit_amd.h
@@ -115,6 +115,12 @@
                                   double lo, double hi, const float *table, int min_block, int num_blocks, int flags,
                                   float *Q, uint8_t *idx, float *E_out, float *row_err, void *workspace, size_t ws_bytes,
                                   slk_stream_t stream);
+
+int slk_gptq_quantize_layers(const float *const *W, const float *const *scale, const long long *const *order,
+                             const double *const *U, const float *const *H, float damp, const float *const *gscale,
+                             int group_size, int batch, int rows_per_layer, int n, int levels, double lo, double hi,
+                             const float *table, int min_block, int num_blocks, int flags, float *Q, uint8_t *idx,
+                             float *E_out, float *row_err, void *workspace, size_t ws_bytes, slk_stream_t stream);
 
 int slk_gptq_quantize_grouped(const float *W, const float *gscale, int group_size, const long long *order, const double *U,
                               int R, int n, int levels, double lo, double hi, const float *table, int min_block,
diff --git a/sleekit_amd/_lib.py b/sleekit_amd/_lib.py
--- a/sleekit_amd/_lib.py
+++ b/sleekit_amd/_lib.py
@@ -69,6 +69,10 @@
     "slk_gptq_quantize_batch_error": (
         c_int,
         [P, P, P, P, P, c_float, c_int, c_int, c_int, c_int, c_double, c_double, P, c_int, c_int, c_int, P, P, P, P, P, c_size_t, P],
+    ),
+    "slk_gptq_quantize_layers": (
+        c_int,
+        [P, P, P, P, P, c_float, P, c_int, c_int, c_int, c_int, c_int, c_double, c_double, P, c_int, c_int, c_int, P, P, P, P, P, c_size_t, P],
     ),
     "slk_gptq_quantize_grouped": (
         c_int,
diff --git a/sleekit_amd/csrc/common.h b/sleekit_amd/csrc/common.h
--- a/sleekit_amd/csrc/common.h
+++ b/sleekit_amd/csrc/common.h
@@ -95,6 +95,17 @@
     const float *p[64];
 };
 
+constexpr int LOOP_LAYERS = 16;
+struct LayerTable {
+    const float *W[LOOP_LAYERS], *scale[LOOP_LAYERS];
+    const long long *order[LOOP_LAYERS];
+    const double *U[LOOP_LAYERS];
+};
+template <class T>
+__device__ __forceinline__ const T *layer_base(const T *const (&column)[LOOP_LAYERS], int b, size_t stride) {
+    return column[b % LOOP_LAYERS] + (size_t)(b - b % LOOP_LAYERS) * stride;
+}
+
 int row_errors_products(const float *W, const float *Q, const float *const *Hs, int batch, int rpl, int n, const int *sym_known,
                         float *row_err, float *G, void *workspace, size_t ws_bytes, slk_stream_t stream);
 
diff --git a/sleekit_amd/csrc/gptq.hip b/sleekit_amd/csrc/gptq.hip
--- a/sleekit_amd/csrc/gptq.hip
+++ b/sleekit_amd/csrc/gptq.hip
@@ -46,17 +46,18 @@
 }
 
 template <bool LDS>
-__global__ __launch_bounds__(256) void k_permute_in(const float *__restrict__ W, const float *__restrict__ scale,
-                                                    const long long *__restrict__ order, int R, int n,
-                                                    float *__restrict__ Qp, int *__restrict__ inv_order, int rpl) {
+__global__ __launch_bounds__(256) void k_permute_in(LayerTable lt, int R, int n, float *__restrict__ Qp,
+                                                    int *__restrict__ inv_order, int rpl) {
     extern __shared__ __attribute__((aligned(16))) float rowbuf[];
     constexpr int V = LDS ? 4 : 1;
     const int t = threadIdx.x;
+    const bool scale = lt.scale[0] != nullptr, order = lt.order[0] != nullptr;
     for (int r = blockIdx.x; r < R; r += gridDim.x) {
-        const float *src = W + (size_t)r * n;
-        const long long *ord = (LDS || order) ? order + (size_t)(r / rpl) * n : nullptr;
+        const int b = r / rpl, rl = r - b * rpl;
+        const float *__restrict__ src = layer_base(lt.W, b, (size_t)rpl * n) + (size_t)rl * n;
+        const long long *__restrict__ ord = (LDS || order) ? layer_base(lt.order, b, n) : nullptr;
         stage_row<LDS>(rowbuf, src, n);
-        const float s = scale ? scale[r] : 1.0f;
+        const float s = scale ? layer_base(lt.scale, b, rpl)[rl] : 1.0f;
         for (int c = V * t; c < n; c += V * 256) {
             long long from[V];
             float v[V];
@@ -70,12 +71,14 @@
             store_elems<V>(Qp + (size_t)r * n + c, v);
         }
     }
-    for (int b = blockIdx.x; b < (R + rpl - 1) / rpl; b += gridDim.x)
-        for (int c = t; c < n; c += 256) inv_order[(size_t)b * n + (order ? order[(size_t)b * n + c] : c)] = c;
+    for (int b = blockIdx.x; b < (R + rpl - 1) / rpl; b += gridDim.x) {
+        const long long *__restrict__ ord = order ? layer_base(lt.order, b, n) : nullptr;
+        for (int c = t; c < n; c += 256) inv_order[(size_t)b * n + (ord ? ord[c] : c)] = c;
+    }
 }
 
 struct RowErrArgs {
-    const float *W, *E, *scale, *hmean;
+    const float *E, *hmean;
     float damp;
     float *row_err;
 };
@@ -84,7 +87,7 @@
     for (int off = 32; off > 0; off >>= 1) v += __shfl_down(v, off, 64);
     return v;
 }
-__device__ __forceinline__ void row_error_store(double se, double sd, double *red, const RowErrArgs &a, int r, int rpl) {
+__device__ __forceinline__ void row_error_store(double se, double sd, double *red, const RowErrArgs &a, int r, int rpl, float scale) {
     se = wave_sum_f64(se);
     sd = wave_sum_f64(sd);
     const int t = threadIdx.x;
@@ -95,7 +98,7 @@
     __syncthreads();
     if (t == 0) {
         const double SE = ((red[0] + red[1]) + red[2]) + red[3], SD = ((red[4] + red[5]) + red[6]) + red[7];
-        const double s = a.scale ? (double)a.scale[r] : 1.0;
+        const double s = (double)scale;
         const float lambda = a.damp * a.hmean[64 * (r / rpl)];
         a.row_err[r] = (float)((s * s) * SE - (double)lambda * SD);
     }
@@ -104,16 +107,19 @@
 
 template <bool LDS, bool ERR>
 __global__ __launch_bounds__(256) void k_permute_out(const float *__restrict__ Qp, const int *__restrict__ inv_order,
-                                                     int R, int n, Grid g, const float *__restrict__ unscale,
-                                                     float *__restrict__ Q, uint8_t *__restrict__ idx, int rpl, RowErrArgs ea) {
+                                                     int R, int n, Grid g, int unscale, float *__restrict__ Q,
+                                                     uint8_t *__restrict__ idx, int rpl, RowErrArgs ea, LayerTable lt) {
     extern __shared__ __attribute__((aligned(16))) float rowbuf[];
     __shared__ double red[ERR ? 8 : 1];
     constexpr int V = LDS ? 4 : 1;
     for (int r = blockIdx.x; r < R; r += gridDim.x) {
         const float *src = Qp + (size_t)r * n;
-        const int *inv_o = inv_order + (size_t)(r / rpl) * n;
+        const int b = r / rpl, rl = r - b * rpl;
+        const int *inv_o = inv_order + (size_t)b * n;
         stage_row<LDS>(rowbuf, src, n);
-        const float inv = unscale ? 1.0f / unscale[r] : 1.0f;
+        const float scale = unscale ? layer_base(lt.scale, b, rpl)[rl] : 1.0f;
+        const float inv = unscale ? 1.0f / scale : 1.0f;
+        const float *__restrict__ wrow = ERR ? layer_base(lt.W, b, (size_t)rpl * n) + (size_t)rl * n : nullptr;
         double se = 0.0, sd = 0.0;
         for (int j = V * threadIdx.x; j < n; j += V * 256) {
             float qw[V];
@@ -131,7 +137,7 @@
             }
             if constexpr (ERR) {
                 float w[V], ev[V];
-                load_elems<V>(ea.W + (size_t)r * n + j, w);
+                load_elems<V>(wrow + j, w);
                 load_elems<V>(ea.E + (size_t)r * n + j, ev);
 #pragma unroll
                 for (int e = 0; e < V; ++e) {
@@ -141,7 +147,7 @@
                 }
             }
         }
-        if constexpr (ERR) row_error_store(se, sd, red, ea, r, rpl);
+        if constexpr (ERR) row_error_store(se, sd, red, ea, r, rpl, scale);
     }
 }
 template <class K, class... A>
@@ -267,7 +273,7 @@
 
 template <bool GROUPED, bool OFFSET = false>
 __global__ __launch_bounds__(512) void k_gptq_window(float *__restrict__ Qp, float *__restrict__ Eg,
-                                                     const double *__restrict__ U, int R, int n, int w0, int w1,
+                                                     LayerTable lt, int R, int n, int w0, int w1,
                                                      Grid g, float inv_step, int fast_ok, int dbg, OpTable tab, int rpl,
                                                      const float *__restrict__ Sg, const int *__restrict__ pg, int G,
                                                      const float *__restrict__ Og) {
@@ -281,7 +287,7 @@
     const bool helper = wave >= 4;
     const int ht = t - 256;
     const int r0 = blockIdx.x * RB;
-    U += (size_t)(r0 / rpl) * n * n;
+    const double *__restrict__ U = layer_base(lt.U, r0 / rpl, (size_t)n * n);
     if constexpr (GROUPED) pg += (size_t)(r0 / rpl) * n;
     if (g.table) {
         for (int i = t; i < 2 * g.n - 1; i += 512) sm.cbt[i] = g.table[i];
@@ -494,14 +500,14 @@
 }
 
 template <bool GROUPED, bool OFFSET = false>
-__global__ __launch_bounds__(512) void k_gptq_wide_leaf(float *__restrict__ Qp, float *__restrict__ Eg, const double *__restrict__ U,
+__global__ __launch_bounds__(512) void k_gptq_wide_leaf(float *__restrict__ Qp, float *__restrict__ Eg, LayerTable lt,
                                                         int R, int n, int a, int b, Grid g, int rpl, const float *__restrict__ Sg,
                                                         const int *__restrict__ pg, int G, const float *__restrict__ Og) {
     static_assert(GROUPED || !OFFSET, "offsets come with group scales");
     const int lane = threadIdx.x & 63, wave = threadIdx.x >> 6, l = lane & 31;
     const int r0 = blockIdx.x * RB, row = r0 + 2 * wave + (lane >> 5);
     const bool live = row < R;
-    U += (size_t)(r0 / rpl) * n * n;
+    const double *__restrict__ U = layer_base(lt.U, r0 / rpl, (size_t)n * n);
     if constexpr (GROUPED) pg += (size_t)(r0 / rpl) * n;
     float *qrow = Qp + (size_t)min(row, R - 1) * n, *erow = Eg + (size_t)min(row, R - 1) * n;
     for (int i = a; i < b; ++i) {
@@ -530,7 +536,7 @@
 }
 
 __global__ __launch_bounds__(256) void k_gptq_trailing(float *__restrict__ Qp, const float *__restrict__ Eg,
-                                                       const double *__restrict__ U, int R, int n, int ka, int kb,
+                                                       LayerTable lt, int R, int n, int ka, int kb,
                                                        int ja, int jb, int vec_ok, int rpl) {
 #ifdef SLK_TRAILING_F64_IMAGE
     __shared__ __attribute__((aligned(16))) Tile64Smem sm;
@@ -538,7 +544,7 @@
     __shared__ __attribute__((aligned(16))) Tile64SmemAf sm;
 #endif
     const int r0 = blockIdx.y * TILE, j0 = ja + blockIdx.x * TILE;
-    U += (size_t)(r0 / rpl) * n * n;
+    const double *__restrict__ U = layer_base(lt.U, r0 / rpl, (size_t)n * n);
     const int t = threadIdx.x;
     Acc64 acc;
     acc.zero();
@@ -747,33 +753,47 @@
     return sizeof(WindowSmem) + (OFFSET ? sizeof(GroupSlots) : GROUPED ? sizeof(GroupTile) : 0);
 }
 template <bool GROUPED, bool OFFSET>
-static int launch_window(double flops, double bytes, int row_tiles, hipStream_t s, float *Qp, float *Eg, const double *U, int R, int n,
-                         int w0, int w1, Grid g, float inv_step, int fast_ok, int dbg, const OpTable &tab, int rpl, const float *Sg,
+static int launch_window(double flops, double bytes, int row_tiles, hipStream_t s, float *Qp, float *Eg, const LayerTable &lt, int R,
+                         int n, int w0, int w1, Grid g, float inv_step, int fast_ok, int dbg, const OpTable &tab, int rpl, const float *Sg,
                          const int *pg, int G, const float *Og) {
     if (w1 - w0 > WMAX) {
         SLK_REQUIRE(tab.count == 1 && tab.op[0].kind == OP_LEAF, "a window of %d columns that is not one leaf", w1 - w0);
         SLK_RUN(OFFSET ? "gptq_window_wide_grouped_asym" : GROUPED ? "gptq_window_wide_grouped" : "gptq_window_wide", flops, bytes, s,
-                k_gptq_wide_leaf<GROUPED, OFFSET><<<row_tiles, 512, 0, s>>>(Qp, Eg, U, R, n, w0, w1, g, rpl, Sg, pg, G, Og));
+                k_gptq_wide_leaf<GROUPED, OFFSET><<<row_tiles, 512, 0, s>>>(Qp, Eg, lt, R, n, w0, w1, g, rpl, Sg, pg, G, Og));
         return SLK_OK;
     }
     SLK_RUN(OFFSET ? "gptq_window_grouped_asym" : GROUPED ? "gptq_window_grouped" : "gptq_window", flops, bytes, s,
-            k_gptq_window<GROUPED, OFFSET><<<row_tiles, 512, window_lds<GROUPED, OFFSET>(), s>>>(Qp, Eg, U, R, n, w0, w1, g, inv_step, fast_ok, dbg,
+            k_gptq_window<GROUPED, OFFSET><<<row_tiles, 512, window_lds<GROUPED, OFFSET>(), s>>>(Qp, Eg, lt, R, n, w0, w1, g, inv_step, fast_ok, dbg,
                                                                                                tab, rpl, Sg, pg, G, Og));
     return SLK_OK;
 }
 
-static int gptq_loop(const float *W, const float *scale, const long long *order, const double *U, int batch, int rows_per_layer,
-                     int n, int levels, double lo, double hi, const float *table, int min_block, int num_blocks, int flags,
-                     float *Q, uint8_t *idx, float *E_out, void *workspace, size_t ws_bytes, slk_stream_t stream,
+static LayerTable stacked_layers(const float *W, const float *scale, const long long *order, const double *U, int batch,
+                                 int rows_per_layer, int n) {
+    LayerTable lt{};
+    for (int b = 0; b < batch && b < LOOP_LAYERS; ++b) {
+        lt.W[b] = W + (size_t)b * rows_per_layer * n;
+        lt.scale[b] = scale ? scale + (size_t)b * rows_per_layer : nullptr;
+        lt.order[b] = order ? order + (size_t)b * n : nullptr;
+        lt.U[b] = U + (size_t)b * n * n;
+    }
+    return lt;
+}
+
+static int gptq_loop(const LayerTable &lt, int batch, int rows_per_layer, int n, int levels, double lo, double hi, const float *table,
+                     int min_block, int num_blocks, int flags, float *Q, uint8_t *idx, float *E_out, void *workspace, size_t ws_bytes, slk_stream_t stream,
                      const float *gscale, int group_size, const float *goffset, const float *const *Hs = nullptr, float damp = 0.0f,
                      float *row_err = nullptr) {
     const bool grouped = gscale != nullptr, asym = goffset != nullptr;
     const int unscale = flags & SLK_LOOP_UNSCALE;
+    const bool scale = lt.scale[0] != nullptr, order = lt.order[0] != nullptr;
     SLK_REQUIRE(!unscale || scale, "unscale needs the row scales");
     SLK_REQUIRE(rows_per_layer > 0 && n > 0, "empty layer");
     SLK_REQUIRE(batch >= 1 && batch <= 64, "batch must be 1..64");
     SLK_REQUIRE(batch == 1 || rows_per_layer % TILE == 0, "a batch needs rows_per_layer to be a multiple of 64");
     SLK_REQUIRE(batch == 1 || order, "a batch needs the column orders");
+    uintptr_t W_bits = 0, U_bits = 0;
+    for (int b = 0; b < batch && b < LOOP_LAYERS; ++b) W_bits |= (uintptr_t)lt.W[b], U_bits |= (uintptr_t)lt.U[b];
     SLK_REQUIRE((long long)batch * rows_per_layer <= 0x7fffffffLL, "too many rows");
     const int R = batch * rows_per_layer, rpl = rows_per_layer;
     SLK_REQUIRE(levels >= 2 && (table || lo < hi), "codebook needs levels >= 2 and lo < hi");
@@ -810,20 +830,20 @@
     SLK_LDS_OPT_IN(k_gptq_window2<2>, sizeof(Window2SmemT<2>));
     const int window_rows = opt(OPT_WINDOW_ROWS) == 16 || opt(OPT_WINDOW_ROWS) == 32 ? opt(OPT_WINDOW_ROWS)
                                                                                      : (((flags & SLK_LOOP_LATENCY) || R < 2048) ? 16 : 32);
-    const bool periods_ok = !grouped && n % 2 == 0 && n <= 16384 && (uintptr_t)U % 16 == 0 && !opt(OPT_NO_WINDOW2) && (dbg & ~(24 | 64 | 128)) == 0;
-
-    const bool perm_lds = order && n % 4 == 0 && n <= PERM_MAX && ((uintptr_t)W | (uintptr_t)Q | (uintptr_t)workspace) % 16 == 0 &&
+    const bool periods_ok = !grouped && n % 2 == 0 && n <= 16384 && U_bits % 16 == 0 && !opt(OPT_NO_WINDOW2) && (dbg & ~(24 | 64 | 128)) == 0;
+
+    const bool perm_lds = order && n % 4 == 0 && n <= PERM_MAX && (W_bits | (uintptr_t)Q | (uintptr_t)workspace) % 16 == 0 &&
                           (idx == nullptr || (uintptr_t)idx % 4 == 0);
     {
-        const int rc = launch_permute("permute_in", 0, 8.0 * R * n, perm_lds ? k_permute_in<true> : k_permute_in<false>, perm_lds, R, n, s, W, scale,
-                                      order, R, n, Qp, inv_order, rpl);
+        const int rc = launch_permute("permute_in", 0, 8.0 * R * n, perm_lds ? k_permute_in<true> : k_permute_in<false>, perm_lds, R, n, s, lt, R,
+                                      n, Qp, inv_order, rpl);
         if (rc != SLK_OK) return rc;
     }
 
     const int G = grouped ? n / group_size : 0;
     if (grouped)
         SLK_RUN("group_of_column", 0, 12.0 * batch * n, s,
-                k_group_of_column<<<(batch * n + 255) / 256, 256, 0, s>>>(order, batch, n, group_size, pg));
+                k_group_of_column<<<(batch * n + 255) / 256, 256, 0, s>>>(lt.order[0], batch, n, group_size, pg));
 
     Plan p;
     plan(0, n, min_block, num_blocks, p);
@@ -868,25 +888,25 @@
                 if (window_rows == 32)
                     SLK_RUN_W("gptq_window", fl * R, wbytes, (R + 2 * RB - 1) / (2 * RB), s,
                               k_gptq_window2<2><<<(R + 2 * RB - 1) / (2 * RB), 512, sizeof(Window2SmemT<2>), s>>>(
-                                  Qp, Eg, U, R, n, st.a, st.b, g, inv_step, fast_ok, dbg & (24 | 64 | 128), pt, rpl));
+                                  Qp, Eg, lt, R, n, st.a, st.b, g, inv_step, fast_ok, dbg & (24 | 64 | 128), pt, rpl));
                 else
                     SLK_RUN_W("gptq_window", fl * R, wbytes, row_tiles, s,
-                              k_gptq_window2<1><<<row_tiles, 512, sizeof(Window2SmemT<1>), s>>>(Qp, Eg, U, R, n, st.a, st.b, g, inv_step,
+                              k_gptq_window2<1><<<row_tiles, 512, sizeof(Window2SmemT<1>), s>>>(Qp, Eg, lt, R, n, st.a, st.b, g, inv_step,
                                                                                              fast_ok, dbg & 24, pt, rpl));
             }
             else {
                 const auto launch = asym ? launch_window<true, true> : grouped ? launch_window<true, false> : launch_window<false, false>;
-                const int rc = launch(fl * R, wbytes, row_tiles, s, Qp, Eg, U, R, n, st.a, st.b, g, inv_step, fast_ok, dbg, tab, rpl, gscale, pg, G,
+                const int rc = launch(fl * R, wbytes, row_tiles, s, Qp, Eg, lt, R, n, st.a, st.b, g, inv_step, fast_ok, dbg, tab, rpl, gscale, pg, G,
                                       goffset);
                 if (rc != SLK_OK) return rc;
             }
         } else {
             const double K = st.b - st.a, N = st.c - st.b;
-            const int vec_ok = n % 4 == 0 && st.a % 4 == 0 && st.b % 2 == 0 && (uintptr_t)U % 16 == 0;
+            const int vec_ok = n % 4 == 0 && st.a % 4 == 0 && st.b % 2 == 0 && U_bits % 16 == 0;
             {
                 dim3 grid((st.c - st.b + TILE - 1) / TILE, (R + TILE - 1) / TILE);
                 SLK_RUN("gptq_trailing", 2.0 * R * K * N, 4.0 * R * K + 8.0 * K * N + 8.0 * R * N, s,
-                        k_gptq_trailing<<<grid, 256, 0, s>>>(Qp, Eg, U, R, n, st.a, st.b, st.b, st.c, vec_ok, rpl));
+                        k_gptq_trailing<<<grid, 256, 0, s>>>(Qp, Eg, lt, R, n, st.a, st.b, st.b, st.c, vec_ok, rpl));
             }
         }
     }
@@ -903,13 +923,13 @@
         if (row_err) {
             const int rc = loop_error_means(Hs, batch, n, hmean, s);
             if (rc != SLK_OK) return rc;
-            ea = RowErrArgs{W, Eg, unscale ? scale : nullptr, hmean, damp, row_err};
+            ea = RowErrArgs{Eg, hmean, damp, row_err};
         }
         const auto kernel = row_err ? (perm_lds ? k_permute_out<true, true> : k_permute_out<false, true>)
                                     : (perm_lds ? k_permute_out<true, false> : k_permute_out<false, false>);
         const int rc = launch_permute(row_err ? "permute_out_error" : "permute_out", row_err ? 4.0 * R * n : 0,
                                       (row_err ? (idx ? 17.0 : 16.0) : (idx ? 9.0 : 8.0)) * R * n, kernel, perm_lds, R, n, s, Qp, inv_order, R, n, g,
-                                      unscale ? scale : nullptr, Q, idx, rpl, ea);
+                                      unscale, Q, idx, rpl, ea, lt);
         if (rc != SLK_OK) return rc;
     }
     if (E_out) copy_async(E_out, Eg, sizeof(float) * (size_t)R * n, s);
@@ -922,8 +942,8 @@
                                        float *E_out, void *workspace, size_t ws_bytes, slk_stream_t stream) {
     SLK_REQUIRE(W && U && Q, "null pointer");
     SLK_REQUIRE((flags & ~(SLK_LOOP_UNSCALE | SLK_LOOP_LATENCY)) == 0, "unknown flags");
-    return gptq_loop(W, scale, order, U, batch, rows_per_layer, n, levels, lo, hi, table, min_block, num_blocks, flags, Q, idx, E_out,
-                     workspace, ws_bytes, stream, nullptr, 0, nullptr);
+    return gptq_loop(stacked_layers(W, scale, order, U, batch, rows_per_layer, n), batch, rows_per_layer, n, levels, lo, hi, table,
+                     min_block, num_blocks, flags, Q, idx, E_out, workspace, ws_bytes, stream, nullptr, 0, nullptr);
 }
 
 extern "C" int slk_gptq_quantize_batch_error(const float *W, const float *scale, const long long *order, const double *U,
@@ -937,8 +957,30 @@
     for (int b = 0; b < batch; ++b) SLK_REQUIRE(H[b] != nullptr, "null Hessian (layer %d)", b);
     SLK_REQUIRE(scale == nullptr || (flags & SLK_LOOP_UNSCALE),
                 "the carried error is that of the de-scaled Q: row scales need SLK_LOOP_UNSCALE");
-    return gptq_loop(W, scale, order, U, batch, rows_per_layer, n, levels, lo, hi, table, min_block, num_blocks, flags, Q, idx, E_out,
-                     workspace, ws_bytes, stream, nullptr, 0, nullptr, H, damp, row_err);
+    return gptq_loop(stacked_layers(W, scale, order, U, batch, rows_per_layer, n), batch, rows_per_layer, n, levels, lo, hi, table,
+                     min_block, num_blocks, flags, Q, idx, E_out, workspace, ws_bytes, stream, nullptr, 0, nullptr, H, damp, row_err);
+}
+
+extern "C" int slk_gptq_quantize_layers(const float *const *W, const float *const *scale, const long long *const *order,
+                                        const double *const *U, const float *const *H, float damp, const float *const *gscale,
+                                        int group_size, int batch, int rows_per_layer, int n, int levels, double lo, double hi,
+                                        const float *table, int min_block, int num_blocks, int flags, float *Q, uint8_t *idx,
+                                        float *E_out, float *row_err, void *workspace, size_t ws_bytes, slk_stream_t stream) {
+    SLK_REQUIRE(W && order && U && Q, "null pointer");
+    SLK_REQUIRE(gscale == nullptr && group_size == 0,
+                "group scales are not taken per layer: stack the layers (slk_gptq_quantize_grouped_batch)");
+    SLK_REQUIRE((flags & ~(SLK_LOOP_UNSCALE | SLK_LOOP_LATENCY)) == 0, "unknown flags");
+    SLK_REQUIRE(batch >= 1 && batch <= LOOP_LAYERS, "the layer table holds 1..%d layers (batch %d)", LOOP_LAYERS, batch);
+    SLK_REQUIRE((H == nullptr) == (row_err == nullptr), "the carried error needs both the Hessians and row_err");
+    SLK_REQUIRE(!H || scale == nullptr || (flags & SLK_LOOP_UNSCALE),
+                "the carried error is that of the de-scaled Q: row scales need SLK_LOOP_UNSCALE");
+    LayerTable lt{};
+    for (int b = 0; b < batch; ++b) {
+        SLK_REQUIRE(W[b] && order[b] && U[b] && (!scale || scale[b]) && (!H || H[b]), "null pointer (layer %d)", b);
+        lt.W[b] = W[b], lt.scale[b] = scale ? scale[b] : nullptr, lt.order[b] = order[b], lt.U[b] = U[b];
+    }
+    return gptq_loop(lt, batch, rows_per_layer, n, levels, lo, hi, table, min_block, num_blocks, flags, Q, idx, E_out, workspace,
+                     ws_bytes, stream, nullptr, 0, nullptr, H, damp, row_err);
 }
 
 static int check_grouped(bool tables, const float *W, const double *U, const float *Q, int flags, int rows_per_layer, int n, int group_size) {
@@ -955,8 +997,8 @@
                                                double hi, const float *table, int min_block, int num_blocks, int flags, float *Q,
                                                uint8_t *idx, float *E_out, void *workspace, size_t ws_bytes, slk_stream_t stream) {
     if (const int rc = check_grouped(gscale != nullptr, W, U, Q, flags, rows_per_layer, n, group_size)) return rc;
-    return gptq_loop(W, nullptr, order, U, batch, rows_per_layer, n, levels, lo, hi, table, min_block, num_blocks, flags, Q, idx, E_out,
-                     workspace, ws_bytes, stream, gscale, group_size, nullptr);
+    return gptq_loop(stacked_layers(W, nullptr, order, U, batch, rows_per_layer, n), batch, rows_per_layer, n, levels, lo, hi, table,
+                     min_block, num_blocks, flags, Q, idx, E_out, workspace, ws_bytes, stream, gscale, group_size, nullptr);
 }
 
 extern "C" int slk_gptq_quantize_grouped(const float *W, const float *gscale, int group_size, const long long *order, const double *U,
@@ -973,8 +1015,8 @@
                                                     int num_blocks, int flags, float *Q, uint8_t *idx, float *E_out, void *workspace,
                                                     size_t ws_bytes, slk_stream_t stream) {
     if (const int rc = check_grouped(gscale && goffset, W, U, Q, flags, rows_per_layer, n, group_size)) return rc;
-    return gptq_loop(W, nullptr, order, U, batch, rows_per_layer, n, levels, lo, hi, table, min_block, num_blocks, flags, Q, idx, E_out,
-                     workspace, ws_bytes, stream, gscale, group_size, goffset);
+    return gptq_loop(stacked_layers(W, nullptr, order, U, batch, rows_per_layer, n), batch, rows_per_layer, n, levels, lo, hi, table,
+                     min_block, num_blocks, flags, Q, idx, E_out, workspace, ws_bytes, stream, gscale, group_size, goffset);
 }
 
 extern "C" int slk_gptq_quantize_grouped_asym(const float *W, const float *gscale, const float *goffset, int group_size,
diff --git a/sleekit_amd/csrc/window2.h b/sleekit_amd/csrc/window2.h
--- a/sleekit_amd/csrc/window2.h
+++ b/sleekit_amd/csrc/window2.h
@@ -96,7 +96,7 @@
 
 template <int SETS>
 __global__ __launch_bounds__(512) void k_gptq_window2(float *__restrict__ Qp, float *__restrict__ Eg,
-                                                      const double *__restrict__ U, int R, int n, int w0, int w1,
+                                                      LayerTable lt, int R, int n, int w0, int w1,
                                                       Grid g, float inv_step, int fast_ok, int prof, PeriodTable tab, int rpl) {
     extern __shared__ __attribute__((aligned(16))) char smem_raw[];
     Window2SmemT<SETS> &sm = *reinterpret_cast<Window2SmemT<SETS> *>(smem_raw);
@@ -113,7 +113,7 @@
     if (!helper && (prof & 128)) __builtin_amdgcn_s_setprio(3);
     const int ht = role_wave * 64 + lane;
     const int r0 = blockIdx.x * RBX;
-    U += (size_t)(r0 / rpl) * n * n;
+    const double *__restrict__ U = layer_base(lt.U, r0 / rpl, (size_t)n * n);
     const int np = tab.count;
     const int width = w1 - w0;
     if (g.table) {
diff --git a/sleekit_amd/dist.py b/sleekit_amd/dist.py
--- a/sleekit_amd/dist.py
+++ b/sleekit_amd/dist.py
@@ -109,6 +109,7 @@
         self.group_rows = int(os.environ.get("SLK_GROUP_ROWS", self.group_rows))
         self.short_factor_batch = int(os.environ.get("SLK_SHORT_FACTOR_BATCH", self.short_factor_batch))
         self.short_rows = int(os.environ.get("SLK_SHORT_ROWS", self.short_rows))
+        self.tall_stack = int(os.environ.get("SLK_TALL_STACK", self.tall_stack))
         self.group_wide_rows = int(os.environ.get("SLK_GROUP_WIDE_ROWS", self.group_wide_rows))
         self.group_bytes = int(os.environ.get("SLK_GROUP_BYTES", self.group_bytes))
 
@@ -312,8 +313,7 @@
         return self.local_batch > 1 and not self.wants_local_batch(layer) and R <= 2048 and self._plain_order()
 
     def run_round_stacked(self, round_layers, factors):
-        order = _stack_views([f[0] for f in factors])
-        U = _stack_views([f[1] for f in factors])
+        order, U = [f[0] for f in factors], [f[1] for f in factors]
         info = torch.cat([f[2] for f in factors])
         known = torch.cat([f[3] for f in factors]) if all(len(f) > 3 for f in factors) else None
         return self._run_stacked(round_layers, 0, round_layers[0]["W"].shape[0], order, U, info, known)
@@ -331,6 +331,12 @@
         rows = hi - lo
         Rp = (rows + 127) // 128 * 128
         Hs = [lay["H"] for lay in round_layers]
+        carried = self._carried_error(round_layers)
+        if (rows == Rp and B <= LOOP_LAYERS and round_layers[0].get("gscale") is None and self.moves == 0
+                and (carried == "loop" or not self.with_error)):
+            return self._shards(round_layers, lo, hi, self._loop_layers(round_layers, lo, hi, list(order), list(U), carried == "loop"), info.split(1))
+        if isinstance(order, list):
+            order, U = _stack_views(order), _stack_views(U)
 
         def stacked(key, fill):
             if round_layers[0].get(key) is None:
@@ -340,7 +346,6 @@
         W, sc, S = stacked("W", 0.0), stacked("scale", 1.0), stacked("gscale", 1.0)
         cb = eng.require_uniform(self.quantizer)
         want_idx = cb[0] <= 256
-        carried = self._carried_error(round_layers)
         if self.moves > 0 and S is None:
             Ws = eng.rows_divide(W.view(B * Rp, n), sc.reshape(-1)).view(B, Rp, n) if sc is not None else W
             Q, idx, _, _ = eng.gptq_loop(Ws, cb, order, U, *self.blocks, want_idx=want_idx)
@@ -355,8 +360,38 @@
                                            want_idx=want_idx, unscale=sc is not None, Hs=Hs if carried == "loop" else None, damp=self.damp)
         if self.with_error and err is None:
             err = eng.row_errors_batch(W, Q, Hs, known)
-        return [dict(Q=Q[b, :rows], idx=idx[b, :rows] if want_idx else None, row_err=None if err is None else err[b, :rows], rows=(lo, hi),
-                     info=info[b:b + 1]) for b in range(B)]
+        return self._shards(round_layers, lo, hi, (Q, idx if want_idx else None, err), info.split(1))
+
+    @staticmethod
+    def _shards(round_layers, lo, hi, stacks, infos):
+        Q, idx, err = stacks
+        rows = hi - lo
+        return [dict(Q=Q[b, :rows], idx=None if idx is None else idx[b, :rows], row_err=None if err is None else err[b, :rows],
+                     rows=(lo, hi), info=infos[b]) for b in range(len(round_layers))]
+
+    def _loop_layers(self, stack_layers, lo, hi, orders, Us, carry, latency=False):
+        eng = self.engine
+        cb = eng.require_uniform(self.quantizer)
+        scaled = stack_layers[0].get("scale") is not None
+        Q, idx, _, err = eng.gptq_loop([lay["W"][lo:hi].contiguous() for lay in stack_layers], cb, orders, Us, *self.blocks,
+                                       scale=[lay["scale"][lo:hi].contiguous() for lay in stack_layers] if scaled else None,
+                                       want_idx=cb[0] <= 256, unscale=scaled, latency=latency,
+                                       Hs=[lay["H"] for lay in stack_layers] if carry else None, damp=self.damp)
+        return Q, idx, err
+
+    tall_stack = 4
+
+    def wants_tall_stack(self, layer):
+        return (self.tall_stack > 1 and self._plain_order() and self.moves == 0 and layer.get("gscale") is None
+                and layer["W"].shape[0] % 64 == 0 and self._carried_error([layer]) == "loop")
+
+    def run_tall(self, stack_layers, factors):
+        R = stack_layers[0]["W"].shape[0]
+        stacks = self._loop_layers(stack_layers, 0, R, [f[0] for f in factors], [f[1] for f in factors], True, latency=not self.overlap)
+        return self._shards(stack_layers, 0, R, stacks, [f[2] for f in factors])
+
+
+LOOP_LAYERS = 16
 
 
 def _guard_inputs(layers, stream):
@@ -641,6 +676,19 @@
         for st in lstreams:
             st.wait_stream(here)
     batched_rounds = getattr(backend, "_loop_rotation", 0) if side else 0
+    tall = {}
+    if not exchange and hasattr(backend, "run_tall"):
+        per = min(int(backend.tall_stack), LOOP_LAYERS)
+        run, run_key = [], None
+        for l in [l for g in rounds for l in g] + [None]:
+            key = None if l is None or not backend.wants_tall_stack(layers[l]) else (tuple(layers[l]["W"].shape), _layer_kind(layers[l]))
+            if key != run_key or len(run) == per:
+                for m in run:
+                    tall[m] = run if m == run[0] else ()
+                run = []
+            run_key = key
+            if key is not None:
+                run.append(l)
     for gi, members_g in enumerate(groups):
         members = [l for g in members_g for l in rounds[g]]
         lo, hi = row_range(layers[members[0]]["W"].shape[0], rank, size)
@@ -665,6 +713,24 @@
                 out[l] = shard
             continue
         for l in members:
+            if l in tall:
+                stack = tall[l]
+                if not stack:
+                    continue
+                ls = lstreams[l % len(lstreams)] if side else None
+                if not join:
+                    _guard_inputs([layers[m] for m in stack], ls)
+                with on(ls):
+                    for m in stack:
+                        if ready[m] is not None:
+                            ls.wait_event(ready[m])
+                    for m, shard in zip(stack, backend.run_tall([layers[m] for m in stack], [factors[m] for m in stack])):
+                        out[m] = shard
+                    if side:
+                        for m in stack:
+                            for t in factors[m]:
+                                t.record_stream(ls)
+                continue
             layer = layers[l]
             ls = lstreams[l % len(lstreams)] if side else None
             if not join:
diff --git a/sleekit_amd/engine.py b/sleekit_amd/engine.py
--- a/sleekit_amd/engine.py
+++ b/sleekit_amd/engine.py
@@ -122,11 +122,22 @@
 
 def gptq_loop(W, cb_abi, order, U, min_block, num_blocks, scale=None, gscale=None, group_size=None, goffset=None, want_idx=True,
               want_E=False, unscale=False, latency=False, Hs=None, damp=None):
-    lead, n = tuple(W.shape[:-1]), W.shape[-1]
-    B, R = lead if len(lead) == 2 else (1,) + lead
-    assert W.is_contiguous() and U.shape == lead[:-1] + (n, n) and U.is_contiguous()
-    assert order is None or (order.shape == lead[:-1] + (n,) and order.is_contiguous())
-    assert scale is None or (gscale is None and scale.shape == lead and scale.is_contiguous())
+    layers = isinstance(W, (list, tuple))
+    if layers:
+        (R, n), device = W[0].shape, W[0].device
+        B, lead = len(W), (len(W), R)
+        assert gscale is None and len(order) == B and len(U) == B and (scale is None or len(scale) == B)
+        for b in range(B):
+            assert W[b].shape == (R, n) and W[b].dtype == torch.float32 and W[b].is_contiguous()
+            assert order[b].shape == (n,) and order[b].dtype == torch.int64 and order[b].is_contiguous()
+            assert U[b].shape == (n, n) and U[b].dtype == torch.float64 and U[b].is_contiguous()
+            assert scale is None or (scale[b].shape == (R,) and scale[b].dtype == torch.float32 and scale[b].is_contiguous())
+    else:
+        lead, n, device = tuple(W.shape[:-1]), W.shape[-1], W.device
+        B, R = lead if len(lead) == 2 else (1,) + lead
+        assert W.is_contiguous() and U.shape == lead[:-1] + (n, n) and U.is_contiguous()
+        assert order is None or (order.shape == lead[:-1] + (n,) and order.is_contiguous())
+        assert scale is None or (gscale is None and scale.shape == lead and scale.is_contiguous())
     assert (gscale is None) == (group_size is None) and (goffset is None or gscale is not None)
     g = 0
     if gscale is not None:
@@ -137,22 +148,28 @@
         assert len(Hs) == B and damp is not None and (scale is None or unscale)
         assert all(H.shape == (n, n) and H.dtype == torch.float32 and H.is_contiguous() for H in Hs)
     ws, ws_bytes = dev.workspace(R, n, batch=B, grouped=gscale is not None and len(lead) == 2)
-    Q = torch.empty_like(W, dtype=torch.float32)
-    idx = torch.empty(W.shape, dtype=torch.uint8, device=W.device) if want_idx else None
+    Q = torch.empty(lead + (n,), dtype=torch.float32, device=device)
+    idx = torch.empty(lead + (n,), dtype=torch.uint8, device=device) if want_idx else None
     E = torch.empty_like(Q) if want_E else None
-    row_err = torch.empty(lead, dtype=torch.float32, device=W.device) if Hs is not None else None
+    row_err = torch.empty(lead, dtype=torch.float32, device=device) if Hs is not None else None
     levels, lo, hi, table = cb_abi
-    factor = (dev.ptr(order), dev.ptr(U))
+
+    def pointers(tensors):
+        return None if tensors is None else (ctypes.c_void_p * B)(*[dev.ptr(t) for t in tensors])
+
+    factor = (pointers(order), pointers(U)) if layers else (dev.ptr(order), dev.ptr(U))
     rest = (B, R, n, levels, lo, hi, dev.ptr(table), int(min_block), int(num_blocks), (1 if unscale else 0) | (2 if latency else 0),
             dev.ptr(Q), dev.ptr(idx), dev.ptr(E))
     end = (dev.ptr(ws), ws_bytes, dev.stream_handle())
-    if goffset is not None:
+    if layers:
+        rc = _lib.lib.slk_gptq_quantize_layers(pointers(W), pointers(scale), *factor, pointers(Hs), float(damp or 0.0), None, 0, *rest,
+                                               dev.ptr(row_err), *end)
+    elif goffset is not None:
         rc = _lib.lib.slk_gptq_quantize_grouped_asym_batch(dev.ptr(W), dev.ptr(gscale), dev.ptr(goffset), g, *factor, *rest, *end)
     elif gscale is not None:
         rc = _lib.lib.slk_gptq_quantize_grouped_batch(dev.ptr(W), dev.ptr(gscale), g, *factor, *rest, *end)
     elif Hs is not None:
-        ptrs = (ctypes.c_void_p * B)(*[dev.ptr(H) for H in Hs])
-        rc = _lib.lib.slk_gptq_quantize_batch_error(dev.ptr(W), dev.ptr(scale), *factor, ptrs, float(damp), *rest, dev.ptr(row_err), *end)
+        rc = _lib.lib.slk_gptq_quantize_batch_error(dev.ptr(W), dev.ptr(scale), *factor, pointers(Hs), float(damp), *rest, dev.ptr(row_err), *end)
     else:
         rc = _lib.lib.slk_gptq_quantize_batch(dev.ptr(W), dev.ptr(scale), *factor, *rest, *end)
     _lib.check(rc)
```

After: 6358 Mweights/s (median of 6 runs). +14.3%, better.
